# bamert/openGPC

Hardware: AMD Instinct MI355X
Metric: Mpix/s hashed+matched (1024x436 pair) (higher is better)
Workload: dtype u8; 1 GPU; BASELINE configs[1] pairs (1024x436, defaultZeroForest.txt, sparsematch settings: thr 5, epipolar, sort-match) in batches of 256 pairs per GPU per step (configs[3] sharding: pair i -> GPU i mod N); width=1024, height=436, tests=30, forest_type=0, parallelism=pairs-dp1, streams_per_gpu=1

## Files before the change

opengpc_amd/csrc/gpc_hip.hip:

```cpp
#include "../../include/gpc_hip.h"

#include <hip/hip_runtime.h>

#if defined(__SSE2__)
#include <emmintrin.h>
#endif
#include <sched.h>

#include <algorithm>
#include <cctype>
#include <condition_variable>
#include <cstdio>
#include <cstdlib>
#include <cstring>
#include <ctime>
#include <deque>
#include <map>
#include <utility>
#include <mutex>
#include <string>
#include <thread>
#include <vector>

#include "gpc_device.h"
// ... 98 lines not shown
class ExpandPool {
 public:
  ~ExpandPool() { stop(); }
  void start(int nthreads, const cpu_set_t* bind, const std::vector<cpu_set_t>* groups = nullptr) {
    if ((int)threads_.size() == nthreads) return;
    stop();
    quit_ = false;
    have_bind_ = bind != nullptr;
    if (bind) bind_ = *bind;
    groups_.clear();
    if (bind && groups) groups_ = *groups;
    cpus_.assign((size_t)nthreads, -1);
    for (int i = 0; i < nthreads; ++i)
      threads_.emplace_back([this, i] {
        if (!groups_.empty()) (void)sched_setaffinity(0, sizeof(cpu_set_t), &groups_[(size_t)i % groups_.size()]);
        else if (have_bind_) (void)sched_setaffinity(0, sizeof bind_, &bind_);
        run(i);
      });
  }
  void stop() {
    {
      std::lock_guard<std::mutex> g(m_);
      quit_ = true;
    }
    cv_.notify_all();
    for (auto& t : threads_) t.join();
    threads_.clear();
  }
  void push(const ExpandJob& j) {
    {
      std::lock_guard<std::mutex> g(m_);
      q_.push_back(j);
      ++pending_[j.slot & 7];
    }
    cv_.notify_one();
  }
  void wait_slot(int slot) {
    std::unique_lock<std::mutex> g(m_);
    done_.wait(g, [&] { return pending_[slot & 7] == 0; });
  }
  void wait_all() {
    for (int s = 0; s < 8; ++s) wait_slot(s);
  }
  int size() const { return (int)threads_.size(); }
  int worker_cpus(int* out, int cap) {
    std::lock_guard<std::mutex> g(m_);
    int n = 0;
    for (size_t i = 0; i < cpus_.size() && n < cap; ++i) out[n++] = cpus_[i];
    return (int)cpus_.size();
  }

 private:
  void run(int index);
  std::vector<std::thread> threads_;
  std::vector<int> cpus_;
  std::deque<ExpandJob> q_;
  std::mutex m_;
  std::condition_variable cv_, done_;
  int pending_[8] = {0, 0, 0, 0, 0, 0, 0, 0};
  bool quit_ = false;
  bool have_bind_ = false;
  cpu_set_t bind_;
  std::vector<cpu_set_t> groups_;
};

}

struct gpc_hip_ctx {
  int device = 0;
  hipStream_t own_stream = nullptr;
  hipStream_t stream = nullptr;
  hipStream_t s_in = nullptr, s_out = nullptr, s_cnt = nullptr;
  hipStream_t s_aux = nullptr;
  hipEvent_t e_fork = nullptr, e_join = nullptr;
  hipEvent_t e_flag = nullptr;
  hipEvent_t e_in[4] = {}, e_comp[4] = {}, e_cnt[4] = {}, e_out[4] = {};
  DevBuf packed;
  void* h_stage = nullptr;
  size_t h_stage_cap = 0;
  void* h_in = nullptr;
  size_t h_in_cap = 0;
  int32_t* h_cnt = nullptr;
  size_t h_cnt_cap = 0;
  ExpandPool pool;
  float stage_ms[4] = {0.f, 0.f, 0.f, 0.f};
  bool grad_is_bits = false;
  bool no_grad_bits = false;
  int upload_mode = 1;
  int direct_max = 2;
  bool have_node_cpus = false;
  cpu_set_t node_cpus;
  std::vector<cpu_set_t> node_l3;
  int numa_node = -1;
  struct Lane {
    hipStream_t s = nullptr;
    hipEvent_t e_in = nullptr, e_hash = nullptr, e_join = nullptr;
    DevBuf smooth, grad, codes, stats, jstate, staged, rowcnt;
    size_t jstate_granules = 0;
    uint32_t join_epoch = 0;
    bool grad_is_bits = false, used = false;
  };
  Lane lanes[2];
  int pipeline = 1, next_lane = 0;
  hipEvent_t dbg_wait_pre = nullptr, dbg_wait_hash = nullptr, dbg_rec_hash = nullptr, dbg_rec_join = nullptr;
  bool no_pair_packed = false;
  bool no_feeder = false;
  int fed_calls = 0;
  int chunk_pairs = 0;
  int expand_threads = 0;
  char err[256] = {0};

  bool naive = false;
  bool have_forest = false;
  GpcForestDev forest;
  GpcForestDev forest_naive;
  int forest_w = 0, forest_h = 0;
  gpc_filter_mask forest_src;
  int ngroups = 0;
  int gmax_tests = 0;
  bool gtau = false;
  DevBuf gforest_dev;
  DevBuf vstats, vcand, vout, vcnt, vncand, uplane, ublk, gdense;
  DevBuf all_rec, all_cnt;
  DevBuf stage;
  hipEvent_t e_stage[2] = {};
  DevBuf tr_plane, tr_pred, tr_blk;
  DevBuf cs_key, cs_idx, cs_cur, cs_start, cs_blk, cs_keep;
  DevBuf py_img, py_rec, py_cnt, py_plane, py_flags, py_blk;
  DevBuf sstats;

  DevBuf raw, smooth, grad, candmap, codes, staged, rowcnt, stats, out, counts, ncand, mask;
  DevBuf gkv;
  DevBuf gkeys[2], gvals[2], ghist, gmisc, hkeys[2], hvals[2], hrec;
  DevBuf gpart;
  int32_t* h_flag = nullptr;
  int no_partition = 0;
  int rows_per_chunk = 16;
  int gp_log2bins = 0;
  int ht_hint_w = 0, ht_hint_h = 0, ht_hint_lbits = 0;
  bool ht_no_half = false;
  int ht_mid = 0;
  int ht_lbits = 0;
  int gp_target = 2000;
  int flat_chunks = 0;
  DevBuf forest_dev;
  int hash_tall = -1;

  DevBuf jstate;
  size_t jstate_granules = 0;
  uint32_t join_epoch = 0;
  int32_t* h_err = nullptr;
  int32_t* d_err = nullptr;
  int no_fuse = 0;
  int fuse_always = 0;
  int fuse_wgs = 0;
  int fuse_min_pairs = 1;
  int pre_rows = 0;
  int fuse_shards = 0;
  int num_cus = 0;
  std::map<std::pair<const void*, size_t>, int> wgs_per_cu;
  std::map<const void*, int> dyn_lds;

  int hash_tpw = 0;
  int join_nt = 0;

  char launch_name[KID_COUNT][96] = {{0}};

  bool timing = false;
  unsigned timing_mask = 0xFFFFFFFFu;
  std::vector<TimedSpan> spans;
  std::vector<TimedSpan> free_spans;

  std::vector<gpc_hip_train_set*> train_sets;
  std::vector<gpc_hip_track_stream*> track_streams;
  uint64_t code_gen = 1;
  DevBuf ext_raw, ext_smooth, ext_grad, ext_groups;
  int extract_frames = 0;
  int seq_frames = 0;

  struct Resident {
    bool valid = false;
    const uint8_t *smooth = nullptr, *grad = nullptr;
    const int32_t* mask = nullptr;
    int n_mask = 0, W = 0, H = 0;
    bool naive = false;
    uint64_t fp = 0;
  };
  Resident res[2];
  int res_next = 0;
  DevBuf res_smooth, res_grad;
  size_t res_n = 0;
  int resident_mode = 1;
  int resident_hits = 0;
  uint8_t* h_xfer = nullptr;
  size_t h_xfer_cap = 0;
  uint8_t* h_pre = nullptr;
  size_t h_pre_cap = 0;
  int pre_slot = -1, pre_W = 0, pre_H = 0;
  bool pre_have_mask = false;
  hipEvent_t e_pre = nullptr;
  struct PendingMatch {
    bool active = false, direct = false, have_ncand = false;
    void* dev_out = nullptr;
    bool packed = false;
    size_t esz = 0;
    int cap_dev = 0, H = 0;
  } pend;
  bool debug = false;
  bool debug_plan = false;
};

struct gpc_hip_train_set {
  gpc_hip_ctx* owner = nullptr;
  int n = 0;
  long np = 0;
  uint8_t* planes = nullptr;
  uint8_t* flags = nullptr;
  int32_t* counts = nullptr;
  gpc::GpcSplit* d_cand = nullptr;
  size_t counts_cap = 0, cand_cap = 0;
  std::vector<int32_t> h_counts;
};

namespace {

std::mutex g_res_mu;
std::vector<gpc_hip_ctx*> g_ctxs;

#define HIPCHK(ctx, call)                                                              \
  do {                                                                                 \
    hipError_t e_ = (call);                                                            \
    if (e_ != hipSuccess) {                                                            \
      snprintf((ctx)->err, sizeof((ctx)->err), "%s failed: %s (%s:%d)", #call,        \
               hipGetErrorString(e_), __FILE__, __LINE__);                             \
      return GPC_E_HIP;                                                                \
    }                                                                                  \
  } while (0)

#define CHK(expr)                  \
  do {                             \
    int s_ = (expr);               \
    if (s_ != GPC_OK) return s_;   \
  } while (0)

double host_ms() {
  timespec ts;
  clock_gettime(CLOCK_MONOTONIC, &ts);
  return ts.tv_sec * 1e3 + ts.tv_nsec * 1e-6;
}

int ensure(gpc_hip_ctx* c, DevBuf& b, size_t bytes) {
  if (bytes <= b.cap) return GPC_OK;
  if (b.p) {
    HIPCHK(c, hipStreamSynchronize(c->stream));
    HIPCHK(c, hipFree(b.p));
    b.p = nullptr;
    b.cap = 0;
  }
  size_t want = bytes + bytes / 8 + 65536;
  HIPCHK(c, hipMalloc(&b.p, want));
  b.cap = want;
  return GPC_OK;
}

void release(DevBuf& b) {
  if (b.p) (void)hipFree(b.p);
  b.p = nullptr;
  b.cap = 0;
}

struct Timed {
  gpc_hip_ctx* c;
  TimedSpan s;
  bool on;
  Timed(gpc_hip_ctx* ctx, int kid) : c(ctx), on(ctx->timing && (kid >= 32 || ((ctx->timing_mask >> kid) & 1u))) {
    if (!on) return;
    if (!c->free_spans.empty()) {
      s = c->free_spans.back();
      c->free_spans.pop_back();
    } else {
      if (hipEventCreate(&s.a) != hipSuccess || hipEventCreate(&s.b) != hipSuccess) {
        on = false;
        return;
      }
    }
    s.kid = kid;
    (void)hipEventRecord(s.a, c->stream);
  }
  ~Timed() {
    if (!on) return;
    (void)hipEventRecord(s.b, c->stream);
    c->spans.push_back(s);
  }
};

int allow_dyn_lds(gpc_hip_ctx* c, const void* fn, size_t bytes) {
  int& have = c->dyn_lds[fn];
  if ((int)bytes <= have) return GPC_OK;
  HIPCHK(c, hipFuncSetAttribute(fn, hipFuncAttributeMaxDynamicSharedMemorySize, (int)bytes));
  have = (int)bytes;
  return GPC_OK;
}

int check_dims(int W, int H) {
  if (W <= 0 || H <= 0 || (W % 16) != 0) return GPC_E_INVALID;
  if (W < 2 * GPC_R + 16 || H < 2 * GPC_R + 4) return GPC_E_INVALID;
// ... 118 lines not shown
  const __m128i m16 = _mm_set1_epi32(0xFFFF);
#endif
  for (int y = y0; y < y1 && pos < limit; ++y) {
    const long cnt = rows[y];
    long n = cnt;
    if (pos + n > limit) n = limit - pos;
    long i = 0;
    auto one = [&](uint32_t v) {
      const int xl = (int)(v & 0xFFFFu), xr = (int)(v >> 16);
      out[pos].x = xl;
      out[pos].y = y;
      out[pos].d = (float)(xl - xr);
      ++pos;
    };
#if defined(__SSE2__)
    if (aligned) {
      for (; i < n && (pos & 3); ++i) one(src[i]);
      const __m128 Y = _mm_castsi128_ps(_mm_set1_epi32(y));
      for (; i + 4 <= n; i += 4, pos += 4) {
        const __m128i v = _mm_loadu_si128(reinterpret_cast<const __m128i*>(src + i));
        const __m128i xl = _mm_and_si128(v, m16);
        const __m128 X = _mm_castsi128_ps(xl);
        const __m128 D = _mm_cvtepi32_ps(_mm_sub_epi32(xl, _mm_srli_epi32(v, 16)));
        const __m128 t0 = _mm_castsi128_ps(_mm_unpacklo_epi32(xl, _mm_castps_si128(Y)));
        const __m128 t1 = _mm_castsi128_ps(_mm_unpackhi_epi32(xl, _mm_castps_si128(Y)));
        const __m128 a = _mm_shuffle_ps(t0, _mm_shuffle_ps(D, X, _MM_SHUFFLE(1, 1, 0, 0)), _MM_SHUFFLE(2, 0, 1, 0));
        const __m128 b = _mm_shuffle_ps(_mm_shuffle_ps(Y, D, _MM_SHUFFLE(1, 1, 0, 0)), t1, _MM_SHUFFLE(1, 0, 2, 0));
        const __m128 c = _mm_shuffle_ps(_mm_shuffle_ps(D, X, _MM_SHUFFLE(3, 3, 2, 2)),
                                        _mm_shuffle_ps(Y, D, _MM_SHUFFLE(3, 3, 0, 0)), _MM_SHUFFLE(2, 0, 2, 0));
        __m128i* o = reinterpret_cast<__m128i*>(out + pos);
        _mm_stream_si128(o, _mm_castps_si128(a));
        _mm_stream_si128(o + 1, _mm_castps_si128(b));
        _mm_stream_si128(o + 2, _mm_castps_si128(c));
      }
    }
#endif
    for (; i < n; ++i) one(src[i]);
    src += cnt;
  }
#if defined(__SSE2__)
  _mm_sfence();
#endif
}

void ExpandPool::run(int index) {
  for (;;) {
    ExpandJob j;
    {
      std::unique_lock<std::mutex> g(m_);
      cv_.wait(g, [&] { return quit_ || !q_.empty(); });
      if (q_.empty()) return;
      j = q_.front();
      q_.pop_front();
      cpus_[(size_t)index] = sched_getcpu();
    }
    if (j.copy_bytes) memcpy(j.copy_dst, j.copy_src, j.copy_bytes);
    else expand_rows(j.packed, j.rows, j.y0, j.y1, j.first, j.limit, j.out);
    {
      std::lock_guard<std::mutex> g(m_);
      if (--pending_[j.slot & 7] == 0) done_.notify_all();
    }
  }
}

int pow2_at_least(int v) {
  int p = 2;
  while (p < v) p <<= 1;
  return p;
}


bool next_tok(const char*& p, std::string& tok) {
  while (*p && isspace((unsigned char)*p)) ++p;
  if (!*p) return false;
  const char* s = p;
  while (*p && !isspace((unsigned char)*p)) ++p;
  tok.assign(s, p - s);
  return true;
}

bool next_int(const char*& p, int& v) {
  std::string tok;
  if (!next_tok(p, tok)) return false;
  char* end = nullptr;
  long l = strtol(tok.c_str(), &end, 10);
  if (end == tok.c_str()) return false;
  v = (int)l;
  return true;
}


int run_global_match(gpc_hip_ctx* c, int W, int H, int npairs, const gpc_settings* s, int mode, const uint8_t* d_cand,
                     void* d_out, int cap, int32_t* d_counts, int32_t* d_ncand, bool seq = false);
int run_hashtable_match(gpc_hip_ctx* c, int W, int H, int npairs, const gpc_settings* s, int mode, const uint8_t* d_cand,
                        void* d_out, int cap, int32_t* d_counts, int32_t* d_ncand, bool seq = false);

int run_preprocess(gpc_hip_ctx* c, const uint8_t* d_raw0, const uint8_t* d_raw1, int W, int H,
                   int npairs, int sides, int thr, bool gradbits = false, uint8_t* d_smooth_out = nullptr,
                   uint8_t* d_grad_out = nullptr, int32_t* d_stats = nullptr) {
  const int nimg = npairs * sides;
  const size_t n = (size_t)W * H;
  if (!d_smooth_out) {
    CHK(ensure(c, c->smooth, n * nimg));
    CHK(ensure(c, c->grad, n * nimg));
    d_smooth_out = (uint8_t*)c->smooth.p;
    d_grad_out = (uint8_t*)c->grad.p;
  } else {
    gradbits = false;
  }
  if (!d_stats) {
    CHK(ensure(c, c->stats, sizeof(int32_t) * GPC_STAT_STRIDE * nimg));
    d_stats = (int32_t*)c->stats.p;
  }
  const int thr_sq = c->naive ? (thr & 0xFF) * (thr & 0xFF) : (int)(int16_t)(uint16_t)((thr & 0xFF) * (thr & 0xFF));
  const int gx = (W / PP_PX + PP_TX - 1) / PP_TX;
  auto blocks_with = [&](int r) { return (long)gx * ((H + PP_TY * r - 1) / (PP_TY * r)) * nimg; };
  int rows = c->pre_rows;
  if (!rows) {
    static const int heights[] = {PP_ROWS, 10, 7, PP_ROWS_MID, 4, PP_ROWS_SMALL};
    const long places = 8l * (c->num_cus > 0 ? c->num_cus : 256);
    long best = -1;
    for (int r : heights) {
      const long cost = (blocks_with(r) + places - 1) / places * (r + 4);
      if (best < 0 || cost < best) { best = cost; rows = r; }
    }
  }
  dim3 grid(gx, (H + PP_TY * rows - 1) / (PP_TY * rows), nimg);
  Timed t(c, KID_PREPROCESS);
  c->grad_is_bits = gradbits && !c->naive && !c->no_grad_bits;
  snprintf(c->launch_name[KID_PREPROCESS], sizeof c->launch_name[0], "gpc::k_preprocess<%s, %d%s>", c->naive ? "true" : "false", rows,
           c->grad_is_bits ? ", true" : "");
#define LAUNCH_PRE(NAIVE, ROWS, BITS)                                                                        \
  hipLaunchKernelGGL((gpc::k_preprocess<NAIVE, ROWS, BITS>), grid, dim3(PP_TX * PP_TY), 0, c->stream, d_raw0, d_raw1, \
                     d_smooth_out, d_grad_out, W, H, sides, thr_sq, d_stats)
#define LAUNCH_PRE_ROWS(NAIVE, BITS)                                  \
  do {                                                                \
    if (rows == PP_ROWS) LAUNCH_PRE(NAIVE, PP_ROWS, BITS);            \
    else if (rows == 10) LAUNCH_PRE(NAIVE, 10, BITS);                 \
    else if (rows == 7) LAUNCH_PRE(NAIVE, 7, BITS);                   \
    else if (rows == PP_ROWS_MID) LAUNCH_PRE(NAIVE, PP_ROWS_MID, BITS); \
    else if (rows == 4) LAUNCH_PRE(NAIVE, 4, BITS);                   \
    else LAUNCH_PRE(NAIVE, PP_ROWS_SMALL, BITS);                      \
  } while (0)
  if (c->naive) LAUNCH_PRE_ROWS(true, false);
  else if (c->grad_is_bits) LAUNCH_PRE_ROWS(false, true);
  else LAUNCH_PRE_ROWS(false, false);
#undef LAUNCH_PRE_ROWS
#undef LAUNCH_PRE
  HIPCHK(c, hipGetLastError());
  return GPC_OK;
}

int run_hash(gpc_hip_ctx* c, const uint8_t* d_smooth, const uint8_t* d_grad, const uint8_t* d_cand,
             int W, int H, int nimg, bool dense, uint32_t* d_codes, int groups = 0, int gstep = 2, int32_t* d_stats = nullptr) {
  if (!c->have_forest) return GPC_E_NO_FOREST;
  const bool gbits = c->grad_is_bits && d_grad == (const uint8_t*)c->grad.p && !dense && !c->naive && d_cand == nullptr;
  const int slots = 2 * (c->num_cus > 0 ? c->num_cus : 256);
  const int gx = (W + HT_X - 1) / HT_X;
  int ty = HT_Y;
  {
    const long n32 = (long)gx * ((H - 2 * GPC_R + HT_Y - 1) / HT_Y) * nimg, n40 = (long)gx * ((H - 2 * GPC_R + HT_Y_TALL - 1) / HT_Y_TALL) * nimg;
    const long c32 = (n32 + slots - 1) / slots * (HT_Y + 2 * GPC_R), c40 = (n40 + slots - 1) / slots * (HT_Y_TALL + 2 * GPC_R);
    if (gbits && n32 < 2l * slots && c40 < c32) ty = HT_Y_TALL;
    if (gbits && c->hash_tall == 1) ty = HT_Y_TALL;
    if (c->hash_tall == 0) ty = HT_Y;
  }
  const int tiles_y = (H - 2 * GPC_R + ty - 1) / ty;
  int tpw = 1;
  if ((long)gx * tiles_y * nimg >= 2l * slots) {
    double best = 1e30;
    for (int t = 2; t <= 16 && t <= tiles_y; ++t) {
      const long per_col = (tiles_y + t - 1) / t, ncol = (long)gx * nimg;
      const long nwg = per_col * ncol;
      if (nwg * 8 < (long)slots * 7) break;
      const int rem = tiles_y - (int)(per_col - 1) * t;
      const long n_full = (per_col - 1) * ncol, n_rem = ncol;
      const long full_rounds = n_full / slots, full_left = n_full % slots;
      double chain = (double)full_rounds * (t + 0.4);
      long short_left = n_rem;
      if (full_left) {
        const long free_places = slots - full_left;
        const long fit = free_places * (long)((t + 0.4) / (rem + 0.4));
        short_left = n_rem > fit ? n_rem - fit : 0;
        chain += t + 0.4;
      }
      chain += (double)((short_left + slots - 1) / slots) * (rem + 0.4);
      if (chain < best - 1e-9) { best = chain; tpw = t; }
    }
  }
  if (c->hash_tpw > 0) tpw = c->hash_tpw < tiles_y ? c->hash_tpw : tiles_y;
  dim3 grid(gx, (tiles_y + tpw - 1) / tpw, nimg);
  const long nwg_all = (long)grid.x * grid.y * grid.z;
  const int last_from = nwg_all > slots ? (int)(nwg_all - slots) : 0;
  Timed t(c, KID_HASH);
  const bool tau = groups > 0 ? c->gtau : c->forest.type != 0;
  int32_t* st = d_stats ? d_stats : (int32_t*)c->stats.p;
  if (groups > 0) {
    const GpcForestDev* gf = (const GpcForestDev*)c->gforest_dev.p;
    snprintf(c->launch_name[KID_HASH], sizeof c->launch_name[0], "gpc::k_hash_groups<%s, %s, %s, %s, %d>", tau ? "true" : "false",
             dense ? "true" : "false", c->naive ? "true" : "false", gbits ? "true" : "false", ty);
#define LAUNCH_HASH_G(TAU, DENSE, NAIVE, GB, TY, FD)                                                                       \
  hipLaunchKernelGGL((gpc::k_hash_groups<TAU, DENSE, NAIVE, GB, TY>), grid, dim3(HT_THREADS), 0, c->stream, d_smooth, d_grad, \
                     d_cand, d_codes, W, H, gf + (FD) * GPC_MAX_GROUPS, st, tpw, last_from, groups, gstep)
    if (gbits) {
      if (ty == HT_Y_TALL) {
        if (tau) LAUNCH_HASH_G(true, false, false, true, HT_Y_TALL, 2); else LAUNCH_HASH_G(false, false, false, true, HT_Y_TALL, 2);
      } else {
        if (tau) LAUNCH_HASH_G(true, false, false, true, HT_Y, 0); else LAUNCH_HASH_G(false, false, false, true, HT_Y, 0);
      }
    } else if (c->naive) {
      if (tau && dense) LAUNCH_HASH_G(true, true, true, false, HT_Y, 1);
      else if (tau) LAUNCH_HASH_G(true, false, true, false, HT_Y, 1);
      else if (dense) LAUNCH_HASH_G(false, true, true, false, HT_Y, 1);
      else LAUNCH_HASH_G(false, false, true, false, HT_Y, 1);
    } else {
      if (tau && dense) LAUNCH_HASH_G(true, true, false, false, HT_Y, 0);
      else if (tau) LAUNCH_HASH_G(true, false, false, false, HT_Y, 0);
      else if (dense) LAUNCH_HASH_G(false, true, false, false, HT_Y, 0);
      else LAUNCH_HASH_G(false, false, false, false, HT_Y, 0);
    }
#undef LAUNCH_HASH_G
    HIPCHK(c, hipGetLastError());
    return GPC_OK;
  }
  snprintf(c->launch_name[KID_HASH], sizeof c->launch_name[0], "gpc::k_hash<%s, %s, %s, %s, %d>", tau ? "true" : "false",
           dense ? "true" : "false", c->naive ? "true" : "false", gbits ? "true" : "false", ty);
#define LAUNCH_HASH(TAU, DENSE, NAIVE)                                                                    \
  hipLaunchKernelGGL((gpc::k_hash<TAU, DENSE, NAIVE>), grid, dim3(HT_THREADS), 0, c->stream, d_smooth, d_grad, \
                     d_cand, d_codes, W, H, (const GpcForestDev*)c->forest_dev.p + (NAIVE ? 1 : 0), st, tpw, last_from)
  if (gbits) {
#define LAUNCH_HASH_BITS(TAU, TY, FD)                                                                                      \
  hipLaunchKernelGGL((gpc::k_hash<TAU, false, false, true, TY>), grid, dim3(HT_THREADS), 0, c->stream, d_smooth, d_grad, \
                     d_cand, d_codes, W, H, (const GpcForestDev*)c->forest_dev.p + FD, st, tpw, last_from)
    if (ty == HT_Y_TALL) {
      if (tau) LAUNCH_HASH_BITS(true, HT_Y_TALL, 2); else LAUNCH_HASH_BITS(false, HT_Y_TALL, 2);
    } else {
      if (tau) LAUNCH_HASH_BITS(true, HT_Y, 0); else LAUNCH_HASH_BITS(false, HT_Y, 0);
    }
#undef LAUNCH_HASH_BITS
  } else if (c->naive) {
    if (tau && dense) LAUNCH_HASH(true, true, true);
    else if (tau) LAUNCH_HASH(true, false, true);
    else if (dense) LAUNCH_HASH(false, true, true);
    else LAUNCH_HASH(false, false, true);
  } else {
    if (tau && dense) LAUNCH_HASH(true, true, false);
    else if (tau) LAUNCH_HASH(true, false, false);
    else if (dense) LAUNCH_HASH(false, true, false);
    else LAUNCH_HASH(false, false, false);
  }
#undef LAUNCH_HASH
  HIPCHK(c, hipGetLastError());
  return GPC_OK;
}

int code_bits(const gpc_hip_ctx* c) {
  const int T = c->ngroups > 1 ? c->gmax_tests : c->forest.num_tests;
  if (c->naive) return T;
  return T <= 8 ? T : T - 1;
}

bool wide_codes(const gpc_hip_ctx* c) { return c->naive && (c->ngroups > 1 ? c->gmax_tests : c->forest.num_tests) == 32; }

struct JoinPlan {
  int nt, spt, log2s;
  size_t lds;
};

JoinPlan plan_join(const gpc_hip_ctx* c, int W) {
  JoinPlan p;
  p.spt = 1;
  p.nt = 256;
  while (p.spt * p.nt < W && p.spt < 4) p.spt <<= 1;
  while (p.spt * p.nt < W && p.nt < 1024) p.nt <<= 1;
  if (c->join_nt && 4 * c->join_nt >= W) {
    p.nt = c->join_nt;
    p.spt = 1;
    while (p.spt * p.nt < W) p.spt <<= 1;
  }
  while (p.spt * p.nt < W && p.spt < 16) p.spt <<= 1;
  p.log2s = 1;
  while ((1 << p.log2s) < p.nt * p.spt || ((1 << p.log2s) < 2 * (W - 2 * GPC_R) && p.log2s < 14)) ++p.log2s;
  p.lds = ((size_t)8 * ((1u << p.log2s) + 1) + 15) / 16 * 16;
  return p;
}

int check_join_err(gpc_hip_ctx* c) {
#ifdef RJ_DBG_COUNT
  if (c->h_err && c->h_err[1]) {
    fprintf(stderr, "[RJ_DBG_COUNT] look-backs %d, windows with a row that had not published %d, displaced keys that met their copy %d\n", c->h_err[1], c->h_err[2], c->h_err[3]);
    c->h_err[1] = c->h_err[2] = c->h_err[3] = 0;
  }
#endif
  if (c->h_err) {
    const int32_t ep = __atomic_exchange_n(c->h_err, 0, __ATOMIC_ACQ_REL);
    if (ep) {
      snprintf(c->err, sizeof(c->err), "k_row_join_fused: a row waited too long for the rows before it in fused launch %d of this "
               "context (%u launched so far): THAT launch's supports are not to be used; a call that reports this at its start "
               "has queued nothing itself", ep, c->join_epoch);
      return GPC_E_HIP;
    }
  }
  return GPC_OK;
}

int join_shards(const gpc_hip_ctx* c, int npairs) {
  if (c->fuse_shards > 0) return npairs < c->fuse_shards ? npairs : c->fuse_shards;
  return join_shards_auto(npairs);
}

int ensure_join_state(gpc_hip_ctx* c, size_t granules) {
  const size_t tk_bytes = sizeof(uint32_t) * RJ_SHARDS * RJ_TICKET_STRIDE;
  if (!c->h_err) {
    HIPCHK(c, hipHostMalloc((void**)&c->h_err, 64, hipHostMallocMapped));
    memset(c->h_err, 0, 64);
    HIPCHK(c, hipHostGetDevicePointer((void**)&c->d_err, c->h_err, 0));
  }
  if (granules > c->jstate_granules || c->join_epoch >= (1u << 30) - 2u) {
    CHK(ensure(c, c->jstate, tk_bytes + sizeof(unsigned long long) * granules));
    HIPCHK(c, hipMemsetAsync(c->jstate.p, 0, c->jstate.cap, c->stream));
    c->jstate_granules = (c->jstate.cap - tk_bytes) / sizeof(unsigned long long);
    c->join_epoch = 0;
  }
  return GPC_OK;
}

int ensure_flag_event(gpc_hip_ctx* c) {
  if (!c->e_flag) HIPCHK(c, hipEventCreateWithFlags(&c->e_flag, hipEventDisableTiming));
  return GPC_OK;
}

int ensure_aux_stream(gpc_hip_ctx* c) {
  if (c->s_aux) return GPC_OK;
  HIPCHK(c, hipStreamCreateWithFlags(&c->s_aux, hipStreamNonBlocking));
  HIPCHK(c, hipEventCreateWithFlags(&c->e_fork, hipEventDisableTiming));
  HIPCHK(c, hipEventCreateWithFlags(&c->e_join, hipEventDisableTiming));
  return GPC_OK;
}

int run_match(gpc_hip_ctx* c, int W, int H, int npairs, const gpc_settings* s, int mode, const uint8_t* d_cand,
              void* d_out, int cap, int32_t* d_counts, int32_t* d_ncand, const PackedOut* po = nullptr, bool seq = false) {
  const int apply_filter = (mode != 1);
  if (mode == 2 && (s->use_hashtable || !s->epipolar_mode || !po)) return GPC_E_UNSUPPORTED;
  if (seq && (mode == 2 || po)) return GPC_E_UNSUPPORTED;
  if (s->use_hashtable) return run_hashtable_match(c, W, H, npairs, s, mode, d_cand, d_out, cap, d_counts, d_ncand, seq);
  if (s->epipolar_mode) {
    CHK(ensure(c, c->staged, sizeof(uint32_t) * (size_t)W * H * npairs));
    CHK(ensure(c, c->rowcnt, sizeof(int32_t) * (size_t)H * npairs * 2));
    int disp_high = s->disp_high;
    if (apply_filter && s->vertical_tolerance < 0) disp_high = -1;
    const JoinPlan jp = plan_join(c, W);
    if (jp.nt * jp.spt < W) return GPC_E_UNSUPPORTED;
    const size_t flds = RJF_LDS_BYTES(jp.nt * jp.spt);
    bool fuse = !seq && !c->no_fuse && npairs >= c->fuse_min_pairs && jp.spt <= 4 && jp.nt * jp.spt <= 4096 &&
                !(po && po->totals) && (long)npairs * (H - 2 * GPC_R) < (1l << 31) - 65536;
    if (fuse && !c->fuse_always) {
      const long lds_wgs = (long)(160 * 1024 / (flds + 64)), wave_wgs = 32 / (jp.nt / 64);
      const long resident = (long)c->num_cus * (lds_wgs < wave_wgs ? lds_wgs : wave_wgs);
      const long rows_total = (long)npairs * (H - 2 * GPC_R);
      fuse = rows_total >= 4 * resident || (W >= 2048 && rows_total >= 3 * resident);
    }
    if (fuse) {
      const int nrows = H - 2 * GPC_R;
      CHK(check_join_err(c));
      CHK(ensure_join_state(c, (size_t)npairs * nrows));
      const size_t lds = flds;
      gpc::RjfArgs a;
      memset(&a, 0, sizeof a);
      a.codes = (const uint32_t*)c->codes.p;
      a.cand = d_cand;
      a.img_stats = (const int32_t*)c->stats.p;
      a.tickets = (uint32_t*)c->jstate.p;
      a.status = (unsigned long long*)((uint32_t*)c->jstate.p + RJ_SHARDS * RJ_TICKET_STRIDE);
      a.err = c->d_err;
      a.out = d_out;
      a.counts = d_counts;
      a.ncand = d_ncand;
      a.rows_out = po ? po->rows : nullptr;
      a.packed_stride = po ? po->packed_stride : 0l;
      a.rows_stride = po ? po->rows_stride : 0l;
      a.W = W;
      a.H = H;
      a.disp_high = disp_high;
      a.apply_filter = apply_filter;
      a.epoch = ++c->join_epoch;
      a.npairs = npairs;
      a.mode = mode;
      a.cap = cap;
      Timed t(c, KID_ROW_JOIN);
      const bool wide = wide_codes(c);
      snprintf(c->launch_name[KID_ROW_JOIN], sizeof c->launch_name[0], "gpc::k_row_join_fused<%d, %d, %s>", jp.spt, jp.nt,
               wide ? "true" : "false");
      c->launch_name[KID_GATHER_ROWS][0] = 0;
#define LAUNCH_RJF(SPT, NT, WIDE)                                                                               \
  do {                                                                                                          \
    const void* fn_ = reinterpret_cast<const void*>(gpc::k_row_join_fused<SPT, NT, WIDE>);                      \
    int& per_cu = c->wgs_per_cu[std::make_pair(fn_, lds)];                                                      \
    if (per_cu == 0) {                                                                                          \
      if (lds > 48 * 1024) CHK(allow_dyn_lds(c, fn_, lds));                                                     \
      HIPCHK(c, hipOccupancyMaxActiveBlocksPerMultiprocessor(&per_cu, fn_, NT, lds));                           \
      if (per_cu < 1) per_cu = 1;                                                                               \
    }                                                                                                           \
     \
    long nwg = c->fuse_wgs > 0 ? c->fuse_wgs : (long)((c->pipeline > 1 && per_cu > 1) ? per_cu - 1 : per_cu) * c->num_cus; \
    if (nwg > (long)npairs * nrows) nwg = (long)npairs * nrows;                                                 \
               \
    int nsh = join_shards(c, npairs);                                                                           \
    if (nsh > nwg) nsh = (int)nwg;                                                                              \
    a.nshards = nsh;                                                                                            \
    if (c->debug) fprintf(stderr, "[gpc_hip] k_row_join_fused<%d, %d>: %d workgroups per CU by the occupancy API, %ld workgroups, %d shards, %zu B of LDS\n", SPT, NT, per_cu, nwg, nsh, lds); \
    const GpcJoinSplit sp_ = make_join_split(npairs, nsh);                                                      \
    a.n_hi = sp_.n_hi;                                                                                          \
    for (int k_ = 0; k_ < 2; ++k_) {                                                                            \
      a.ps[k_] = sp_.ps[k_];                                                                                    \
      a.ps_magic[k_] = sp_.ps_magic[k_];                                                                        \
      a.ps_sh[k_] = sp_.ps_sh[k_];                                                                              \
    }                                                                                                           \
    hipLaunchKernelGGL((gpc::k_row_join_fused<SPT, NT, WIDE>), dim3((unsigned)nwg), dim3(NT), lds, c->stream, a); \
  } while (0)
#define LAUNCH_RJF_W(SPT, NT) do { if (wide) LAUNCH_RJF(SPT, NT, true); else LAUNCH_RJF(SPT, NT, false); } while (0)
#define LAUNCH_RJF_S(NT)                      \
  switch (jp.spt) {                           \
    case 1: LAUNCH_RJF_W(1, NT); break;       \
    case 2: LAUNCH_RJF_W(2, NT); break;       \
    default: LAUNCH_RJF_W(4, NT); break;      \
  }
      if (jp.nt == 1024) { LAUNCH_RJF_S(1024) }
      else if (jp.nt == 512) { LAUNCH_RJF_S(512) }
      else { LAUNCH_RJF_S(256) }
#undef LAUNCH_RJF_S
#undef LAUNCH_RJF_W
#undef LAUNCH_RJF
      HIPCHK(c, hipGetLastError());
      return GPC_OK;
    }
    {
      Timed t(c, KID_ROW_JOIN);
      const int rpw = 1;
      const dim3 jgrid((H - 2 * GPC_R + rpw - 1) / rpw, npairs);
      const bool wide = wide_codes(c);
      snprintf(c->launch_name[KID_ROW_JOIN], sizeof c->launch_name[0], "gpc::k_row_join%s<%d, %d, %s>", seq ? "_seq" : "",
               jp.spt, jp.nt, wide ? "true" : "false");
#define LAUNCH_JOIN_K(K, SPT, NT, WIDE)                                                                       \
  do {                                                                                                        \
    const void* fn_ = reinterpret_cast<const void*>(gpc::K<SPT, NT, WIDE>);                                   \
    if (jp.lds > 48 * 1024) CHK(allow_dyn_lds(c, fn_, jp.lds));                                               \
    hipLaunchKernelGGL((gpc::K<SPT, NT, WIDE>), jgrid, dim3(NT), jp.lds, c->stream,                           \
                       (const uint32_t*)c->codes.p, d_cand, W, H, disp_high, apply_filter,                    \
                       (const int32_t*)c->stats.p, (uint32_t*)c->staged.p, (int32_t*)c->rowcnt.p, jp.log2s,   \
                       rpw, gpc::RjVirt());                                                    \
  } while (0)
#define LAUNCH_JOIN(SPT, NT, WIDE) \
  do { if (seq) LAUNCH_JOIN_K(k_row_join_seq, SPT, NT, WIDE); else LAUNCH_JOIN_K(k_row_join, SPT, NT, WIDE); } while (0)
#define LAUNCH_JOIN_W(SPT, NT) do { if (wide) LAUNCH_JOIN(SPT, NT, true); else LAUNCH_JOIN(SPT, NT, false); } while (0)
#define LAUNCH_JOIN_S(NT)                      \
  switch (jp.spt) {                            \
    case 1: LAUNCH_JOIN_W(1, NT); break;       \
    case 2: LAUNCH_JOIN_W(2, NT); break;       \
    default: LAUNCH_JOIN_W(4, NT); break;      \
  }
      if (jp.nt == 1024) {
        if (jp.spt == 16) LAUNCH_JOIN_W(16, 1024);
        else if (jp.spt == 8) LAUNCH_JOIN_W(8, 1024);
        else LAUNCH_JOIN_S(1024)
      } else if (jp.nt == 512) { LAUNCH_JOIN_S(512) }
      else { LAUNCH_JOIN_S(256) }
#undef LAUNCH_JOIN_S
#undef LAUNCH_JOIN_W
#undef LAUNCH_JOIN
#undef LAUNCH_JOIN_K
      HIPCHK(c, hipGetLastError());
    }
    {
      Timed t(c, KID_GATHER_ROWS);
      snprintf(c->launch_name[KID_GATHER_ROWS], sizeof c->launch_name[0], "gpc::k_gather_rows");
      if (po && po->totals)
        hipLaunchKernelGGL(gpc::k_pair_totals, dim3(npairs), dim3(RM_THREADS), 0, c->stream, (const int32_t*)c->rowcnt.p, H,
                           po->totals);
      const int gr = ((long)((H - 2 * GPC_R + GR_ROWS - 1) / GR_ROWS) * npairs >= 2048) ? GR_ROWS : 1;
      hipLaunchKernelGGL(gpc::k_gather_rows, dim3((H - 2 * GPC_R + gr - 1) / gr, npairs), dim3(RM_THREADS), 0, c->stream,
                         (const uint32_t*)c->staged.p, (const int32_t*)c->rowcnt.p, W, H, mode, d_out,
                         cap, d_counts, (const int32_t*)c->stats.p, d_ncand, gr, po ? po->rows : nullptr,
                         po ? po->packed_stride : 0l, po ? po->rows_stride : 0l,
                         po ? (const int32_t*)po->totals : (const int32_t*)nullptr);
      HIPCHK(c, hipGetLastError());
    }
    return GPC_OK;
  }
  return run_global_match(c, W, H, npairs, s, mode, d_cand, d_out, cap, d_counts, d_ncand, seq);
}

struct GlobalPlan {
  int nmax, nblk, nmblk;
  gpc::GpcBatchStrides bs;
  int32_t *hist, *blkcnt, *gmisc, *rowcnt;
  size_t esz;
};

int plan_global(gpc_hip_ctx* c, int W, int H, int npairs, int mode, int cap, bool hashtable, GlobalPlan& g, bool seq) {
  const size_t n = (size_t)W * H;
  g.nmax = 2 * (W - 2 * GPC_R) * (H - 2 * GPC_R);
  g.nblk = (g.nmax + GS_TILE - 1) / GS_TILE;
  g.nmblk = (g.nmax + RM_THREADS - 1) / RM_THREADS;
  g.esz = mode == 0 ? sizeof(gpc_support) : sizeof(gpc_correspondence);
  const size_t recs = (size_t)g.nmax * npairs;
  for (int i = 0; i < 2; ++i) {
    CHK(ensure(c, c->gkeys[i], sizeof(uint32_t) * recs));
    CHK(ensure(c, c->gvals[i], sizeof(uint32_t) * recs));
    if (hashtable) {
      CHK(ensure(c, c->hkeys[i], sizeof(uint32_t) * recs));
      CHK(ensure(c, c->hvals[i], sizeof(uint32_t) * recs));
    }
  }
  if (hashtable) CHK(ensure(c, c->hrec, 2 * sizeof(uint32_t) * recs));
  CHK(ensure(c, c->ghist, sizeof(int32_t) * ((size_t)256 * g.nblk + g.nmblk) * npairs));
  CHK(ensure(c, c->gmisc, sizeof(int32_t) * GM_STRIDE * npairs));
  CHK(ensure(c, c->rowcnt, sizeof(int32_t) * (size_t)H * 2 * npairs));
  g.hist = (int32_t*)c->ghist.p;
  g.blkcnt = g.hist + (size_t)256 * g.nblk * npairs;
  g.gmisc = (int32_t*)c->gmisc.p;
  g.rowcnt = (int32_t*)c->rowcnt.p;
  g.bs.codes = (long)((seq ? 1 : 2) * n);
  g.bs.recs = g.nmax;
  g.bs.hist = (long)256 * g.nblk;
  g.bs.blk = g.nmblk;
  g.bs.out = (long)cap * (long)g.esz;
  g.bs.rows = 2 * H;
  return GPC_OK;
}

int radix_passes(gpc_hip_ctx* c, const GlobalPlan& g, int npairs, uint32_t* keys[2], uint32_t* vals[2], int passes) {
  for (int pass = 0; pass < passes; ++pass) {
    const int src = pass & 1, dst = src ^ 1;
    hipLaunchKernelGGL(gpc::k_g_hist, dim3(g.nblk, npairs), dim3(GS_THREADS), 0, c->stream,
                       (const uint32_t*)keys[src], (const int32_t*)g.gmisc, 8 * pass, g.hist, g.nblk, g.bs);
    hipLaunchKernelGGL(gpc::k_g_scan, dim3(1, npairs), dim3(1024), 0, c->stream, g.hist, 256 * g.nblk, g.bs.hist);
    hipLaunchKernelGGL(gpc::k_g_scatter, dim3(g.nblk, npairs), dim3(GS_THREADS), 0, c->stream,
                       (const uint32_t*)keys[src], (const uint32_t*)vals[src], keys[dst], vals[dst],
                       (const int32_t*)g.gmisc, 8 * pass, (const int32_t*)g.hist, g.nblk, g.bs);
  }
  HIPCHK(c, hipGetLastError());
  return GPC_OK;
}

void launch_radix_records(gpc_hip_ctx* c, const GlobalPlan& g, int W, int H, int npairs, const uint8_t* d_cand, uint32_t* keys,
                          uint32_t* vals) {
  const uint32_t* codes = (const uint32_t*)c->codes.p;
  const uint8_t* wcand = wide_codes(c) ? d_cand : nullptr;
  const int32_t* stats = (const int32_t*)c->stats.p;
  const dim3 rgrid(H - 2 * GPC_R, 2, npairs);
  hipLaunchKernelGGL(gpc::k_g_rowcount, rgrid, dim3(RM_THREADS), 0, c->stream, codes, wcand, W, H, g.rowcnt, stats, g.gmisc, g.bs);
  hipLaunchKernelGGL(gpc::k_g_build, rgrid, dim3(RM_THREADS), 0, c->stream, codes, wcand, W, H, (const int32_t*)g.rowcnt, stats,
                     keys, vals, g.gmisc, g.bs);
}

void name_join_launch(gpc_hip_ctx* c, const char* kernel, bool list) {
  char* n = c->launch_name[KID_GLOBAL_MATCH];
  const size_t at = strlen(n);
  snprintf(n + at, sizeof c->launch_name[0] - at, "%s%s%s", at ? " + " : "", kernel, list ? "[list]" : "");
}

struct CodeRangePlan {
  int32_t overflow;
  int32_t max_parts;
  int32_t max_bin_side;
  int32_t max_list;
};
struct BucketCheck {
  int32_t overflow;
  int32_t max_bin;
  int32_t max_pair;
  int32_t max_list;
};
template <class Words>
Words plan_words(const gpc_hip_ctx* c) {
  static_assert(sizeof(Words) == 4 * sizeof(int32_t), "a planner leaves four words");
  Words w;
  memcpy(&w, c->h_flag, sizeof w);
  return w;
}

struct PartIo {
  const uint32_t* codes;
  const uint8_t* wcand;
// ... 640 lines not shown
}

namespace {

int run_group_match(gpc_hip_ctx* c, const uint8_t* d_sm, const uint8_t* d_gr, const uint8_t* d_cand_hash, int W, int H,
                    int npairs, const gpc_settings* s, int mode, const uint8_t* d_cand, void* d_out, long cap,
                    int32_t* d_counts, int32_t* d_ncand) {
  if (s->use_hashtable) return GPC_E_UNSUPPORTED;
  const int G = c->ngroups;
  const size_t n = (size_t)W * H;
  const int npv = npairs * G;
  const size_t esz = mode == 0 ? sizeof(gpc_support) : sizeof(gpc_correspondence);
  const long vcap = (long)(W - 2 * GPC_R) * (H - 2 * GPC_R) + 1;
  CHK(ensure(c, c->codes, sizeof(uint32_t) * n * 2 * npv));
  CHK(ensure(c, c->vstats, sizeof(int32_t) * GPC_STAT_STRIDE * 2 * npv));
  CHK(ensure(c, c->vout, esz * (size_t)vcap * npv));
  CHK(ensure(c, c->vcnt, sizeof(int32_t) * npv));
  CHK(ensure(c, c->vncand, sizeof(int32_t) * 2 * npv));
  hipLaunchKernelGGL(gpc::k_stats_init, dim3((2 * npv + 63) / 64), dim3(64), 0, c->stream, (int32_t*)c->vstats.p, 2 * npv);
  std::swap(c->stats, c->vstats);
  int st = run_hash(c, d_sm, d_gr, d_cand_hash, W, H, 2 * npairs, false, (uint32_t*)c->codes.p, G, 2);
  const uint8_t* vc = d_cand;
  if (st == GPC_OK && wide_codes(c) && d_cand) {
    st = ensure(c, c->vcand, 2 * n * npv);
    for (int p = 0; p < npairs && st == GPC_OK; ++p)
      for (int g = 0; g < G && st == GPC_OK; ++g)
        if (hipMemcpyAsync((uint8_t*)c->vcand.p + (size_t)(p * G + g) * 2 * n, d_cand + (size_t)p * 2 * n, 2 * n,
                           hipMemcpyDeviceToDevice, c->stream) != hipSuccess)
          st = GPC_E_HIP;
    vc = (const uint8_t*)c->vcand.p;
  }
  if (st == GPC_OK)
    st = run_match(c, W, H, npv, s, mode, vc, c->vout.p, (int)vcap, (int32_t*)c->vcnt.p, (int32_t*)c->vncand.p);
  std::swap(c->stats, c->vstats);
  CHK(st);
  const int nchunk = (int)((vcap + UN_CHUNK - 1) / UN_CHUNK);
  CHK(ensure(c, c->uplane, sizeof(uint32_t) * n * npv));
  CHK(ensure(c, c->ublk, sizeof(int32_t) * (size_t)nchunk * npv));
  Timed t(c, KID_GROUP_UNION);
  snprintf(c->launch_name[KID_GROUP_UNION], sizeof c->launch_name[0], "gpc::k_group_union<%s>", mode == 0 ? "false" : "true");
  HIPCHK(c, hipMemsetAsync(c->uplane.p, 0xFF, sizeof(uint32_t) * n * npv, c->stream));
  const dim3 sgrid(nchunk < 512 ? nchunk : 512, npv), cgrid(nchunk, npv);
#define UNION_LAUNCH(CORR)                                                                                                  \
  do {                                                                                                                     \
    typedef gpc::UnRec<CORR> R_;                                                                                           \
    const R_* vo_ = (const R_*)c->vout.p;                                                                                  \
    hipLaunchKernelGGL((gpc::k_group_union_scatter<CORR>), sgrid, dim3(UN_THREADS), 0, c->stream, vo_,                     \
                       (const int32_t*)c->vcnt.p, vcap, W, H, (uint32_t*)c->uplane.p, G);                                  \
    hipLaunchKernelGGL((gpc::k_group_union_count<CORR>), cgrid, dim3(UN_THREADS), 0, c->stream, vo_,                       \
                       (const int32_t*)c->vcnt.p, vcap, W, H, (const uint32_t*)c->uplane.p, G, (int32_t*)c->ublk.p, nchunk); \
    hipLaunchKernelGGL(gpc::k_group_union_scan, dim3(npairs), dim3(1024), 0, c->stream, (int32_t*)c->ublk.p, nchunk, G,    \
                       d_counts, d_ncand, (const int32_t*)c->vstats.p);                                                    \
    hipLaunchKernelGGL((gpc::k_group_union<CORR>), cgrid, dim3(UN_THREADS), 0, c->stream, vo_, (const int32_t*)c->vcnt.p,  \
                       vcap, W, H, (const uint32_t*)c->uplane.p, G, (const int32_t*)c->ublk.p, nchunk, (R_*)d_out, cap);   \
  } while (0)
  if (mode == 0) UNION_LAUNCH(false);
  else UNION_LAUNCH(true);
#undef UNION_LAUNCH
  HIPCHK(c, hipGetLastError());
  return GPC_OK;
}

}


extern "C" {

int gpc_hip_abi_version(void) { return GPC_HIP_ABI_VERSION; }

const char* gpc_hip_status_string(int status) {
  switch (status) {
    case GPC_OK: return "ok";
    case GPC_E_INVALID: return "invalid argument";
    case GPC_E_NO_DEVICE: return "no usable HIP device (gfx950 required)";
    case GPC_E_HIP: return "HIP runtime error";
    case GPC_E_CAPACITY: return "output capacity too small";
    case GPC_E_NO_FOREST: return "no forest set";
    case GPC_E_FOREST_RANGE: return "forest test offset outside the 27x27 patch";
    case GPC_E_IO: return "forest file could not be read";
    case GPC_E_UNSUPPORTED: return "unsupported setting on the HIP path";
    default: return "unknown status";
  }
}

int gpc_hip_device_count(int* count) {
  if (!count) return GPC_E_INVALID;
  int n = 0;
  if (hipGetDeviceCount(&n) != hipSuccess) {
    *count = 0;
    return GPC_E_NO_DEVICE;
  }
  *count = n;
  return GPC_OK;
}

int gpc_hip_create(int device, gpc_hip_ctx** out) {
  if (!out) return GPC_E_INVALID;
  *out = nullptr;
  int n = 0;
  if (hipGetDeviceCount(&n) != hipSuccess || n <= 0 || device < 0 || device >= n) return GPC_E_NO_DEVICE;
  if (hipSetDevice(device) != hipSuccess) return GPC_E_NO_DEVICE;
  hipDeviceProp_t prop;
  if (hipGetDeviceProperties(&prop, device) != hipSuccess) return GPC_E_NO_DEVICE;
  if (strncmp(prop.gcnArchName, "gfx950", 6) != 0) return GPC_E_NO_DEVICE;
  gpc_hip_ctx* c = new gpc_hip_ctx();
  c->device = device;
  if (hipStreamCreateWithFlags(&c->own_stream, hipStreamNonBlocking) != hipSuccess) {
    delete c;
    return GPC_E_NO_DEVICE;
  }
  c->stream = c->own_stream;
  const char* ht = getenv("GPC_HIP_HASH_TPW");
  if (ht && atoi(ht) > 0 && atoi(ht) <= 64) c->hash_tpw = atoi(ht);
  c->no_partition = getenv("GPC_HIP_NO_PARTITION") != nullptr;
  c->flat_chunks = getenv("GPC_HIP_FLAT_CHUNKS") != nullptr;
  if (const char* e = getenv("GPC_HIP_GP_TARGET")) {
    const int v = atoi(e);
    if (v >= 256 && v <= 3500) c->gp_target = v;
  }
  if (const char* e = getenv("GPC_HIP_GP_LOG2BINS")) {
    const int v = atoi(e);
    if (v >= 8 && v <= 11) c->gp_log2bins = v;
  }
  c->ht_no_half = getenv("GPC_HIP_HT_NO_HALF") != nullptr;
  if (const char* e = getenv("GPC_HIP_HT_MID")) {
    const int v = atoi(e);
    if (v >= HM_CAP && v <= 64) c->ht_mid = v;
  }
  if (const char* e = getenv("GPC_HIP_HT_LBITS")) {
    const int v = atoi(e);
    if (v >= 7 && v <= 10) c->ht_lbits = v;
  }
  if (const char* e = getenv("GPC_HIP_ROWS_PER_CHUNK")) {
    const int v = atoi(e);
    if (v >= 1 && v <= 64) c->rows_per_chunk = v;
  }
  if (const char* e = getenv("GPC_HIP_DIRECT_MAX")) {
    const int v = atoi(e);
    if (v >= 0 && v <= 4096) c->direct_max = v;
  }
  const char* ck = getenv("GPC_HIP_CHUNK");
  if (ck && atoi(ck) > 0 && atoi(ck) <= 1024) c->chunk_pairs = atoi(ck);
  if (const char* e = getenv("GPC_HIP_SEQ_FRAMES")) {
    const int v = atoi(e);
    if (v >= 2 && v <= 1024) c->seq_frames = v;
  }
  const char* et = getenv("GPC_HIP_EXPAND_THREADS");
  if (et && atoi(et) > 0 && atoi(et) <= 64) c->expand_threads = atoi(et);
  if (const char* e = getenv("GPC_HIP_UPLOAD")) c->upload_mode = atoi(e);
  c->no_grad_bits = getenv("GPC_HIP_NO_GRAD_BITS") != nullptr;
  c->no_feeder = getenv("GPC_HIP_NO_FEEDER") != nullptr;
  c->no_pair_packed = getenv("GPC_HIP_NO_PAIR_PACKED") != nullptr;
  c->no_fuse = getenv("GPC_HIP_NO_FUSE") != nullptr;
  if (const char* e = getenv("GPC_HIP_HASH_TALL")) c->hash_tall = atoi(e) ? 1 : 0;
  if (const char* e = getenv("GPC_HIP_PRE_ROWS")) {
    const int v = atoi(e);
    if (v == PP_ROWS || v == 10 || v == 7 || v == PP_ROWS_MID || v == 4 || v == PP_ROWS_SMALL) c->pre_rows = v;
  }
  c->fuse_always = getenv("GPC_HIP_FUSE_ALWAYS") != nullptr;
  if (const char* e = getenv("GPC_HIP_FUSE_WGS")) {
    const int v = atoi(e);
    if (v >= 1 && v <= 65536) c->fuse_wgs = v;
  }
  if (const char* e = getenv("GPC_HIP_FUSE_SHARDS")) {
    const int v = atoi(e);
    if (v >= 1 && v <= RJ_SHARDS) c->fuse_shards = v;
  }
  if (const char* e = getenv("GPC_HIP_FUSE_MIN_PAIRS")) {
    const int v = atoi(e);
    if (v >= 1) c->fuse_min_pairs = v;
  }
  if (const char* e = getenv("GPC_HIP_RESIDENT")) {
    const int v = atoi(e);
    if (v >= 0 && v <= 2) c->resident_mode = v;
  }
  if (const char* e = getenv("GPC_HIP_EXTRACT_FRAMES")) {
    const int v = atoi(e);
    if (v >= 1) c->extract_frames = v;
  }
  c->debug = getenv("GPC_HIP_DEBUG") != nullptr;
  c->debug_plan = getenv("GPC_HIP_DEBUG_PLAN") != nullptr;
  c->num_cus = prop.multiProcessorCount;
  find_gpu_node_cpus(c);
  const char* jn = getenv("GPC_HIP_JOIN_NT");
  if (jn && (atoi(jn) == 256 || atoi(jn) == 512 || atoi(jn) == 1024)) c->join_nt = atoi(jn);
  {
    std::lock_guard<std::mutex> g(g_res_mu);
    g_ctxs.push_back(c);
  }
  *out = c;
  return GPC_OK;
}

int gpc_hip_destroy(gpc_hip_ctx* c) {
  if (!c) return GPC_E_INVALID;
  {
    std::lock_guard<std::mutex> g(g_res_mu);
    for (size_t k = 0; k < g_ctxs.size(); ++k)
      if (g_ctxs[k] == c) { g_ctxs.erase(g_ctxs.begin() + k); break; }
  }
  (void)hipSetDevice(c->device);
  (void)drain_lanes(c);
  (void)hipStreamSynchronize(c->stream);
  const int pending_err = check_join_err(c);
  if (pending_err != GPC_OK) fprintf(stderr, "gpc_hip_destroy: %s\n", c->err);
  DevBuf* bufs[] = {&c->raw, &c->smooth, &c->grad, &c->candmap, &c->codes, &c->staged, &c->rowcnt,
                    &c->stats, &c->out, &c->counts, &c->ncand, &c->mask, &c->gkeys[0], &c->gkeys[1],
                    &c->gvals[0], &c->gvals[1], &c->ghist, &c->gmisc, &c->hkeys[0], &c->hkeys[1],
                    &c->hvals[0], &c->hvals[1], &c->hrec, &c->forest_dev, &c->packed, &c->gpart, &c->jstate, &c->gkv,
                    &c->res_smooth, &c->res_grad, &c->ext_raw, &c->ext_smooth, &c->ext_grad, &c->ext_groups,
                    &c->sstats, &c->all_rec, &c->all_cnt, &c->stage, &c->tr_plane, &c->tr_pred, &c->tr_blk,
                    &c->cs_key, &c->cs_idx, &c->cs_cur, &c->cs_start, &c->cs_blk, &c->cs_keep,
                    &c->py_img, &c->py_rec, &c->py_cnt, &c->py_plane, &c->py_flags, &c->py_blk};
  while (!c->train_sets.empty()) (void)gpc_hip_train_set_destroy(c, c->train_sets.back());
  while (!c->track_streams.empty()) (void)gpc_hip_track_stream_destroy(c, c->track_streams.back());
  for (DevBuf* b : bufs) release(*b);
  for (auto& s : c->spans) { (void)hipEventDestroy(s.a); (void)hipEventDestroy(s.b); }
  for (auto& s : c->free_spans) { (void)hipEventDestroy(s.a); (void)hipEventDestroy(s.b); }
  if (c->s_in) {
    (void)hipStreamDestroy(c->s_in);
    (void)hipStreamDestroy(c->s_out);
    (void)hipStreamDestroy(c->s_cnt);
    for (int i = 0; i < 4; ++i) {
      (void)hipEventDestroy(c->e_in[i]);
      (void)hipEventDestroy(c->e_comp[i]);
      (void)hipEventDestroy(c->e_cnt[i]);
      (void)hipEventDestroy(c->e_out[i]);
    }
  }
  if (c->e_flag) (void)hipEventDestroy(c->e_flag);
  if (c->e_pre) (void)hipEventDestroy(c->e_pre);
  for (hipEvent_t e : c->e_stage)
    if (e) (void)hipEventDestroy(e);
  for (auto& l : c->lanes) {
    if (l.s) {
      (void)hipStreamSynchronize(l.s);
      (void)hipStreamDestroy(l.s);
      (void)hipEventDestroy(l.e_in);
      (void)hipEventDestroy(l.e_hash);
      (void)hipEventDestroy(l.e_join);
    }
    DevBuf* lb[] = {&l.smooth, &l.grad, &l.codes, &l.stats, &l.jstate, &l.staged, &l.rowcnt};
    for (DevBuf* b : lb) release(*b);
  }
  if (c->s_aux) {
    (void)hipStreamDestroy(c->s_aux);
    (void)hipEventDestroy(c->e_fork);
    (void)hipEventDestroy(c->e_join);
  }
  c->pool.stop();
  if (c->h_stage) (void)hipHostFree(c->h_stage);
  if (c->h_in) (void)hipHostFree(c->h_in);
  if (c->h_cnt) (void)hipHostFree(c->h_cnt);
  if (c->h_pre) (void)hipHostFree(c->h_pre);
  if (c->h_xfer) (void)hipHostFree(c->h_xfer);
  if (c->h_flag) (void)hipHostFree(c->h_flag);
  if (c->h_err) (void)hipHostFree(c->h_err);
  if (c->own_stream) (void)hipStreamDestroy(c->own_stream);
  delete c;
  return pending_err;
}

const char* gpc_hip_last_error(const gpc_hip_ctx* c) { return c ? c->err : "null context"; }

int gpc_hip_set_stream(gpc_hip_ctx* c, void* hip_stream) {
  if (!c) return GPC_E_INVALID;
  c->stream = hip_stream ? (hipStream_t)hip_stream : c->own_stream;
  return GPC_OK;
}

int gpc_hip_synchronize(gpc_hip_ctx* c) {
  if (!c) return GPC_E_INVALID;
  CHK(drain_lanes(c));
  HIPCHK(c, hipStreamSynchronize(c->stream));
  return check_join_err(c);
}

int gpc_hip_reserve(gpc_hip_ctx* c, int W, int H, int max_pairs) {
  if (!c || max_pairs <= 0) return GPC_E_INVALID;
  CHK(check_dims(W, H));
  HIPCHK(c, hipSetDevice(c->device));
  const size_t n = (size_t)W * H;
  const int nimg = 2 * max_pairs;
  const int G = c->ngroups > 1 ? c->ngroups : 1;
  CHK(ensure(c, c->raw, n * nimg));
  CHK(ensure(c, c->smooth, n * nimg));
  CHK(ensure(c, c->grad, n * nimg));
  CHK(ensure(c, c->codes, sizeof(uint32_t) * n * nimg * G));
  if (G > 1) {
    CHK(ensure(c, c->vstats, sizeof(int32_t) * GPC_STAT_STRIDE * nimg * G));
    CHK(ensure(c, c->vcnt, sizeof(int32_t) * max_pairs * G));
    CHK(ensure(c, c->vncand, sizeof(int32_t) * nimg * G));
    CHK(ensure(c, c->uplane, sizeof(uint32_t) * n * max_pairs * G));
  }
  CHK(ensure(c, c->staged, sizeof(uint32_t) * n * max_pairs));
  CHK(ensure(c, c->rowcnt, sizeof(int32_t) * (size_t)H * nimg));
  CHK(ensure(c, c->stats, sizeof(int32_t) * GPC_STAT_STRIDE * nimg));
  CHK(ensure(c, c->counts, sizeof(int32_t) * nimg));
  CHK(ensure(c, c->ncand, sizeof(int32_t) * nimg));
  return GPC_OK;
}

int gpc_hip_set_arithmetic(gpc_hip_ctx* c, int mode) {
  if (!c || (mode != GPC_ARITH_SSE && mode != GPC_ARITH_NAIVE)) return GPC_E_INVALID;
  if (c->naive != (mode == GPC_ARITH_NAIVE)) ++c->code_gen;
  c->naive = (mode == GPC_ARITH_NAIVE);
// ... 526 lines not shown
    d_sm = (const uint8_t*)c->smooth.p;
    d_gr = (const uint8_t*)c->grad.p;
    d_cand = d_cm;
  }
  c->grad_is_bits = false;
  c->pend.dev_out = nullptr;
  if (groups) {
    const long cap_u = (long)c->ngroups * ((long)(W - 2 * GPC_R) * (H - 2 * GPC_R)) + 1;
    CHK(ensure(c, c->gdense, esz * (size_t)cap_u));
    CHK(run_group_match(c, d_sm, d_gr, resident ? nullptr : d_cand, W, H, 1, s, mode, d_cand, c->gdense.p, cap_u, d_cnt,
                        nullptr));
    cap_dev = (int)std::min(cap_u, (long)INT32_MAX);
    c->pend.dev_out = c->gdense.p;
  } else {
  hipLaunchKernelGGL(gpc::k_stats_init, dim3(1), dim3(64), 0, c->stream, (int32_t*)c->stats.p, 2);
  CHK(run_hash(c, d_sm, d_gr, resident ? nullptr : d_cand, W, H, 2, false, (uint32_t*)c->codes.p));
  if (packed) {
    const PackedOut po = {reinterpret_cast<int32_t*>(d_arena), (long)cap_dev, (long)H};
    CHK(run_match(c, W, H, 1, s, 2, d_cand, d_arena + rows_bytes, cap_dev, d_cnt, nullptr, &po));
  } else {
    CHK(run_match(c, W, H, 1, s, mode, d_cand, d_out, cap_dev, d_cnt, nullptr));
  }
  }
  c->pend.active = true;
  c->pend.direct = direct_out != nullptr;
  c->pend.have_ncand = false;
  c->pend.packed = packed;
  c->pend.esz = esz;
  c->pend.cap_dev = cap_dev;
  c->pend.H = H;
  return GPC_OK;
}

static int match_fetch(gpc_hip_ctx* c, void* out, int cap, int* n_out, int* ncl, int* ncr) {
  if (!c || !c->pend.active || !n_out || cap < 0 || (cap > 0 && !out)) return GPC_E_INVALID;
  HIPCHK(c, hipStreamSynchronize(c->stream));
  CHK(check_join_err(c));
  const int32_t cnt = c->h_cnt[0];
  *n_out = cnt;
  if (c->pend.have_ncand) {
    if (ncl) *ncl = c->h_cnt[1];
    if (ncr) *ncr = c->h_cnt[2];
  }
  int ncopy = cnt < cap ? cnt : cap;
  if (ncopy > c->pend.cap_dev) ncopy = c->pend.cap_dev;
  if (c->pend.dev_out && ncopy > 0) {
    const size_t bytes = c->pend.esz * (size_t)ncopy;
    uint8_t* d_arena = nullptr;
    CHK(xfer_reserve(c, bytes, &d_arena));
    HIPCHK(c, hipMemcpyAsync(c->h_xfer, c->pend.dev_out, bytes, hipMemcpyDeviceToHost, c->stream));
    HIPCHK(c, hipStreamSynchronize(c->stream));
    const bool par = bytes >= 256 * 1024;
    if (par) CHK(ensure_pool(c));
    host_copy(c, out, c->h_xfer, bytes, par);
    if (par) host_copy_wait(c);
  } else if (c->pend.packed && ncopy > 0) {
    const int H = c->pend.H;
    const int32_t* rows = reinterpret_cast<const int32_t*>(c->h_xfer);
    const uint32_t* words = reinterpret_cast<const uint32_t*>(c->h_xfer + pad16(sizeof(int32_t) * (size_t)H));
    const bool par = ncopy >= 32 * 1024;
    if (par) CHK(ensure_pool(c));
    const int parts = par ? (c->pool.size() > 1 ? c->pool.size() : 1) : 1;
    long first = 0;
    for (int q = 0; q < parts; ++q) {
      const int y0 = GPC_R + (int)((long)(H - 2 * GPC_R) * q / parts), y1 = GPC_R + (int)((long)(H - 2 * GPC_R) * (q + 1) / parts);
      if (first < ncopy && y1 > y0) {
        if (par) c->pool.push(ExpandJob{words, rows, H, y0, y1, (int)first, ncopy, static_cast<gpc_support*>(out), 6});
        else expand_rows(words, rows, y0, y1, first, ncopy, static_cast<gpc_support*>(out));
      }
      for (int y = y0; y < y1; ++y) first += rows[y];
    }
    if (par) host_copy_wait(c);
  } else if (!c->pend.direct && ncopy > 0) {
    const size_t bytes = c->pend.esz * (size_t)ncopy;
    const bool par = bytes >= 256 * 1024;
    if (par) CHK(ensure_pool(c));
    host_copy(c, out, c->h_xfer, bytes, par);
    if (par) host_copy_wait(c);
  }
  return (cnt > cap || cnt > c->pend.cap_dev) ? GPC_E_CAPACITY : GPC_OK;
}

static int match_preprocessed(gpc_hip_ctx* c, const uint8_t* smoothL, const uint8_t* gradL,
                              const int32_t* maskL, int nL, const uint8_t* smoothR, const uint8_t* gradR,
                              const int32_t* maskR, int nR, int W, int H, const gpc_settings* s, int mode,
                              void* out, int cap, int* n_out) {
  if (!n_out || cap < 0 || (cap > 0 && !out)) return GPC_E_INVALID;
  const size_t esz = mode == 0 ? sizeof(gpc_support) : sizeof(gpc_correspondence);
  void* dv = (c && cap > 0 && (uint64_t)cap * esz < (1ull << 32)) ? device_view_of_host(out) : nullptr;
  CHK(match_preprocessed_begin(c, smoothL, gradL, maskL, nL, smoothR, gradR, maskR, nR, W, H, s, mode, cap, dv));
  const int st = match_fetch(c, out, cap, n_out, nullptr, nullptr);
  c->pend.active = false;
  return st;
}

int gpc_hip_rectified_match(gpc_hip_ctx* c, const uint8_t* smoothL, const uint8_t* gradL,
                            const int32_t* maskL, int nL, const uint8_t* smoothR, const uint8_t* gradR,
                            const int32_t* maskR, int nR, int W, int H, const gpc_settings* s,
                            gpc_support* out, int cap, int* n_out) {
  return match_preprocessed(c, smoothL, gradL, maskL, nL, smoothR, gradR, maskR, nR, W, H, s, 0, out, cap, n_out);
}

int gpc_hip_stereo_match(gpc_hip_ctx* c, const uint8_t* smoothL, const uint8_t* gradL,
                         const int32_t* maskL, int nL, const uint8_t* smoothR, const uint8_t* gradR,
                         const int32_t* maskR, int nR, int W, int H, const gpc_settings* s,
                         gpc_correspondence* out, int cap, int* n_out) {
  return match_preprocessed(c, smoothL, gradL, maskL, nL, smoothR, gradR, maskR, nR, W, H, s, 1, out, cap, n_out);
}

int gpc_hip_rectified_match_begin(gpc_hip_ctx* c, const uint8_t* smoothL, const uint8_t* gradL, const int32_t* maskL, int nL,
                                  const uint8_t* smoothR, const uint8_t* gradR, const int32_t* maskR, int nR, int W, int H,
                                  const gpc_settings* s) {
  return match_preprocessed_begin(c, smoothL, gradL, maskL, nL, smoothR, gradR, maskR, nR, W, H, s, 0, (nL < nR ? nL : nR) + 1, nullptr);
}

int gpc_hip_stereo_match_begin(gpc_hip_ctx* c, const uint8_t* smoothL, const uint8_t* gradL, const int32_t* maskL, int nL,
                               const uint8_t* smoothR, const uint8_t* gradR, const int32_t* maskR, int nR, int W, int H,
                               const gpc_settings* s) {
  return match_preprocessed_begin(c, smoothL, gradL, maskL, nL, smoothR, gradR, maskR, nR, W, H, s, 1, (nL < nR ? nL : nR) + 1, nullptr);
}

int gpc_hip_match_fetch(gpc_hip_ctx* c, void* out, int cap, int* n_out, int* n_cand_l, int* n_cand_r) {
  return match_fetch(c, out, cap, n_out, n_cand_l, n_cand_r);
}


int gpc_hip_match_batch_device(gpc_hip_ctx* c, const uint8_t* d_rawL, const uint8_t* d_rawR, int W, int H,
                               int npairs, const gpc_settings* s, gpc_support* d_out, int cap_per_pair,
                               int32_t* d_counts, int32_t* d_ncand) {
  if (!c || !d_rawL || !d_rawR || !d_out || !d_counts || npairs <= 0 || cap_per_pair <= 0) return GPC_E_INVALID;
  CHK(check_settings(s));
  CHK(check_dims(W, H));
  CHK(forest_matches(c, W, H));
  HIPCHK(c, hipSetDevice(c->device));
  const size_t n = (size_t)W * H;
  if (c->ngroups > 1) {
    if (c->pipeline > 1 || s->use_hashtable) return GPC_E_UNSUPPORTED;
    CHK(run_preprocess(c, d_rawL, d_rawR, W, H, npairs, 2, s->gradient_threshold, true));
    return run_group_match(c, (const uint8_t*)c->smooth.p, (const uint8_t*)c->grad.p, nullptr, W, H, npairs, s, 0,
                           (const uint8_t*)c->grad.p, d_out, cap_per_pair, d_counts, d_ncand);
  }
  if (c->pipeline > 1 && s->epipolar_mode && !s->use_hashtable) {
    CHK(ensure_lanes(c));
    gpc_hip_ctx::Lane& lane = c->lanes[c->next_lane];
    gpc_hip_ctx::Lane& other = c->lanes[c->next_lane ^ 1];
    c->next_lane ^= 1;
    HIPCHK(c, hipEventRecord(lane.e_in, c->stream));
    HIPCHK(c, hipStreamWaitEvent(lane.s, lane.e_in, 0));
    if (other.used) HIPCHK(c, hipStreamWaitEvent(lane.s, other.e_hash, 0));
    LaneScope in(c, lane);
    lane.used = true;
    CHK(ensure(c, c->codes, sizeof(uint32_t) * n * 2 * npairs));
    CHK(run_preprocess(c, d_rawL, d_rawR, W, H, npairs, 2, s->gradient_threshold, true));
    CHK(run_hash(c, (const uint8_t*)c->smooth.p, (const uint8_t*)c->grad.p, nullptr, W, H, 2 * npairs, false, (uint32_t*)c->codes.p));
    HIPCHK(c, hipEventRecord(lane.e_hash, c->stream));
    CHK(run_match(c, W, H, npairs, s, 0, (const uint8_t*)c->grad.p, d_out, cap_per_pair, d_counts, d_ncand));
    HIPCHK(c, hipEventRecord(lane.e_join, c->stream));
    return GPC_OK;
  }
  if (c->pipeline > 1) CHK(drain_lanes(c));
  CHK(ensure(c, c->codes, sizeof(uint32_t) * n * 2 * npairs));
  if (c->dbg_wait_pre) HIPCHK(c, hipStreamWaitEvent(c->stream, c->dbg_wait_pre, 0));
  CHK(run_preprocess(c, d_rawL, d_rawR, W, H, npairs, 2, s->gradient_threshold, true));
  if (c->dbg_wait_hash) HIPCHK(c, hipStreamWaitEvent(c->stream, c->dbg_wait_hash, 0));
  CHK(run_hash(c, (const uint8_t*)c->smooth.p, (const uint8_t*)c->grad.p, nullptr, W, H, 2 * npairs, false,
               (uint32_t*)c->codes.p));
  if (c->dbg_rec_hash) HIPCHK(c, hipEventRecord(c->dbg_rec_hash, c->stream));
  CHK(run_match(c, W, H, npairs, s, 0, (const uint8_t*)c->grad.p, d_out, cap_per_pair, d_counts, d_ncand));
  if (c->dbg_rec_join) HIPCHK(c, hipEventRecord(c->dbg_rec_join, c->stream));
  return GPC_OK;
}

int gpc_hip_set_pipeline(gpc_hip_ctx* c, int lanes) {
  if (!c || (lanes != 1 && lanes != 2)) return GPC_E_INVALID;
  if (lanes == 2 && c->ngroups > 1) return GPC_E_UNSUPPORTED;
  HIPCHK(c, hipSetDevice(c->device));
  CHK(drain_lanes(c));
  HIPCHK(c, hipStreamSynchronize(c->stream));
  c->pipeline = lanes;
  return GPC_OK;
}

int gpc_hip_pipeline_join(gpc_hip_ctx* c) {
  if (!c) return GPC_E_INVALID;
  for (auto& l : c->lanes)
    if (l.s && l.used) HIPCHK(c, hipStreamWaitEvent(c->stream, l.e_join, 0));
  return GPC_OK;
}

int gpc_hip_debug_pipeline_events(gpc_hip_ctx* c, void* wait_before_preprocess, void* wait_before_hash, void* record_after_hash,
                                  void* record_after_join) {
  if (!c) return GPC_E_INVALID;
  c->dbg_wait_pre = (hipEvent_t)wait_before_preprocess;
  c->dbg_wait_hash = (hipEvent_t)wait_before_hash;
  c->dbg_rec_hash = (hipEvent_t)record_after_hash;
  c->dbg_rec_join = (hipEvent_t)record_after_join;
  return GPC_OK;
}

static int batch_streams(gpc_hip_ctx* c) {
  if (c->s_in) return GPC_OK;
  HIPCHK(c, hipStreamCreateWithFlags(&c->s_in, hipStreamNonBlocking));
  HIPCHK(c, hipStreamCreateWithFlags(&c->s_out, hipStreamNonBlocking));
  HIPCHK(c, hipStreamCreateWithFlags(&c->s_cnt, hipStreamNonBlocking));
  for (int i = 0; i < 4; ++i) {
    HIPCHK(c, hipEventCreateWithFlags(&c->e_in[i], hipEventDisableTiming));
    HIPCHK(c, hipEventCreateWithFlags(&c->e_comp[i], hipEventDisableTiming));
    HIPCHK(c, hipEventCreateWithFlags(&c->e_cnt[i], hipEventDisableTiming));
    HIPCHK(c, hipEventCreateWithFlags(&c->e_out[i], hipEventDisableTiming));
  }
  return GPC_OK;
}

static int match_batch_unpacked(gpc_hip_ctx* c, const uint8_t* rawL, const uint8_t* rawR, int W, int H, int npairs,
                                const gpc_settings* s, gpc_support* out, int cap, int32_t* counts, int32_t* ncand) {
  if (!c || !rawL || !rawR || !out || !counts || npairs <= 0 || cap <= 0) return GPC_E_INVALID;
  CHK(check_settings(s));
  CHK(check_dims(W, H));
  CHK(forest_matches(c, W, H));
  HIPCHK(c, hipSetDevice(c->device));
  const size_t n = (size_t)W * H;
  const int chunk = npairs >= 8 ? (npairs >= 32 ? 8 : npairs / 4) : npairs;
  const int nch = (npairs + chunk - 1) / chunk;
  CHK(ensure(c, c->raw, 2 * 2 * n * chunk));
  CHK(ensure(c, c->out, sizeof(gpc_support) * (size_t)cap * npairs));
  CHK(ensure(c, c->counts, sizeof(int32_t) * npairs));
  CHK(ensure(c, c->ncand, sizeof(int32_t) * 2 * npairs));
  CHK(batch_streams(c));
  CHK(pinned_counts(c, npairs));
  const bool bounce = !device_view_of_host(rawL) || !device_view_of_host(rawR);
  const bool land = !device_view_of_host(out);
  if (bounce || land) CHK(ensure_pool(c));
  if (bounce) {
    const size_t need = 2 * 2 * n * (size_t)chunk;
    if (need > c->h_in_cap) {
      HIPCHK(c, hipStreamSynchronize(c->s_in));
      if (c->h_in) HIPCHK(c, hipHostFree(c->h_in));
      c->h_in = nullptr;
      c->h_in_cap = 0;
      HIPCHK(c, hipHostMalloc(&c->h_in, need, hipHostMallocDefault));
      c->h_in_cap = need;
    }
  }
  const size_t slot_bytes = sizeof(gpc_support) * (size_t)cap * chunk;
  if (land && 2 * slot_bytes > c->h_stage_cap) {
    c->pool.wait_all();
    HIPCHK(c, hipStreamSynchronize(c->s_out));
    if (c->h_stage) HIPCHK(c, hipHostFree(c->h_stage));
    c->h_stage = nullptr;
    c->h_stage_cap = 0;
    HIPCHK(c, hipHostMalloc(&c->h_stage, 2 * slot_bytes, hipHostMallocDefault));
    c->h_stage_cap = 2 * slot_bytes;
  }
  int32_t* hc = c->h_cnt;
  int32_t* hn = c->h_cnt + npairs;
  int status = GPC_OK;
  auto collect = [&](int k) -> int {
    const int p0 = k * chunk, pc = (p0 + chunk <= npairs) ? chunk : npairs - p0;
    HIPCHK(c, hipEventSynchronize(c->e_cnt[k & 1]));
    memcpy(counts + p0, hc + p0, sizeof(int32_t) * pc);
    if (ncand) memcpy(ncand + 2 * p0, hn + 2 * p0, sizeof(int32_t) * 2 * pc);
    if (land) c->pool.wait_slot(k & 1);
    gpc_support* lslot = land ? reinterpret_cast<gpc_support*>((uint8_t*)c->h_stage + (size_t)(k & 1) * slot_bytes) : nullptr;
    for (int p = p0; p < p0 + pc; ++p) {
      const int ncopy = counts[p] < cap ? counts[p] : cap;
      if (counts[p] > cap) status = GPC_E_CAPACITY;
      if (ncopy > 0)
        HIPCHK(c, hipMemcpyAsync(land ? lslot + (size_t)(p - p0) * cap : out + (size_t)p * cap,
                                 (gpc_support*)c->out.p + (size_t)p * cap, sizeof(gpc_support) * (size_t)ncopy,
                                 hipMemcpyDeviceToHost, c->s_out));
    }
    if (land) HIPCHK(c, hipEventRecord(c->e_out[k & 1], c->s_out));
    return GPC_OK;
  };
  auto deliver = [&](int k) -> int {
    if (!land) return GPC_OK;
    const int p0 = k * chunk, pc = (p0 + chunk <= npairs) ? chunk : npairs - p0;
    HIPCHK(c, hipEventSynchronize(c->e_out[k & 1]));
    const gpc_support* lslot = reinterpret_cast<const gpc_support*>((uint8_t*)c->h_stage + (size_t)(k & 1) * slot_bytes);
    for (int p = p0; p < p0 + pc; ++p) {
      const int ncopy = counts[p] < cap ? counts[p] : cap;
      const size_t bytes = sizeof(gpc_support) * (size_t)ncopy, step = 256 * 1024;
      for (size_t at = 0; at < bytes; at += step) {
        ExpandJob j = {};
        j.slot = k & 1;
        j.copy_src = reinterpret_cast<const uint8_t*>(lslot + (size_t)(p - p0) * cap) + at;
        j.copy_dst = reinterpret_cast<uint8_t*>(out + (size_t)p * cap) + at;
        j.copy_bytes = at + step <= bytes ? step : bytes - at;
        c->pool.push(j);
      }
    }
    return GPC_OK;
  };
  for (int k = 0; k < nch; ++k) {
    const int slot = k & 1, p0 = k * chunk, pc = (p0 + chunk <= npairs) ? chunk : npairs - p0;
    uint8_t* d_l = (uint8_t*)c->raw.p + (size_t)slot * 2 * n * chunk;
    uint8_t* d_r = d_l + n * chunk;
    if (k >= 2) HIPCHK(c, hipStreamWaitEvent(c->s_in, c->e_comp[slot], 0));
    const uint8_t *srcL = rawL + (size_t)p0 * n, *srcR = rawR + (size_t)p0 * n;
    if (bounce) {
      uint8_t* bl = (uint8_t*)c->h_in + (size_t)slot * 2 * n * chunk;
      uint8_t* br = bl + n * chunk;
      if (k >= 2) HIPCHK(c, hipEventSynchronize(c->e_in[slot]));
      const size_t bytes = n * pc, step = 256 * 1024;
      for (int side = 0; side < 2; ++side)
        for (size_t at = 0; at < bytes; at += step) {
          ExpandJob j = {};
          j.slot = 7;
          j.copy_src = (side ? srcR : srcL) + at;
          j.copy_dst = (side ? br : bl) + at;
          j.copy_bytes = at + step <= bytes ? step : bytes - at;
          c->pool.push(j);
        }
      c->pool.wait_slot(7);
      srcL = bl;
      srcR = br;
    }
    HIPCHK(c, hipMemcpyAsync(d_l, srcL, n * pc, hipMemcpyHostToDevice, c->s_in));
    HIPCHK(c, hipMemcpyAsync(d_r, srcR, n * pc, hipMemcpyHostToDevice, c->s_in));
    HIPCHK(c, hipEventRecord(c->e_in[slot], c->s_in));
    HIPCHK(c, hipStreamWaitEvent(c->stream, c->e_in[slot], 0));
// ... 1363 lines not shown
extern "C++" {
template <bool CORR>
static int pyr_match(gpc_hip_ctx* c, const uint8_t* d_a, const uint8_t* d_b, int W, int H, int npairs, int levels,
                     const gpc_settings* s, void* d_out, int cap, int32_t* d_counts, int32_t* d_level_counts, int32_t* d_ncand) {
  int32_t ws[GPC_MAX_PYRAMID_LEVELS], hs[GPC_MAX_PYRAMID_LEVELS];
  CHK(pyr_usable(c, s, W, H, levels, ws, hs));
  if (npairs > 65535) return GPC_E_UNSUPPORTED;
  if (levels > 1) {
    CHK(gpc::pyr_down_check(d_a, d_out, W, H, CORR ? npairs + 1 : npairs));
    if (!CORR) CHK(gpc::pyr_down_check(d_b, d_out, W, H, npairs));
  }
  HIPCHK(c, hipSetDevice(c->device));
  if (c->pipeline > 1) CHK(drain_lanes(c));
  StrictScope strict(c);
  const int nimg = CORR ? npairs + 1 : npairs;
  const size_t ncs = CORR ? (size_t)nimg : 2 * (size_t)npairs;
  auto match = [&](int l, const uint8_t* a, const uint8_t* b, void* rec, int rcap, int32_t* cnt) -> int {
    const gpc_settings sl = gpc::pyr_level_settings(*s, l);
    int32_t* nc = d_ncand ? d_ncand + (size_t)l * ncs : nullptr;
    LevelScope level(c, ws[l], hs[l]);
    if (CORR) return gpc_hip_match_sequence_device(c, a, ws[l], hs[l], nimg, &sl, (gpc_correspondence*)rec, rcap, cnt, nc);
    return gpc_hip_match_batch_device(c, a, b, ws[l], hs[l], npairs, &sl, (gpc_support*)rec, rcap, cnt, nc);
  };
  if (levels == 1) {
    CHK(match(0, d_a, d_b, d_out, cap, d_counts));
    HIPCHK(c, hipMemcpyAsync(d_level_counts, d_counts, sizeof(int32_t) * (size_t)npairs, hipMemcpyDeviceToDevice, c->stream));
    return GPC_OK;
  }
  const size_t esz = sizeof(gpc::PyRec<CORR>);
  size_t img_at[GPC_MAX_PYRAMID_LEVELS] = {0}, rec_at[GPC_MAX_PYRAMID_LEVELS] = {0}, img_bytes = 0, rec_bytes = 0;
  int32_t caps[GPC_MAX_PYRAMID_LEVELS];
  for (int l = 0; l < levels; ++l) {
    caps[l] = (int32_t)gpc::pyr_level_cap(ws[l], hs[l]);
    rec_at[l] = rec_bytes;
    rec_bytes += pad16(esz * (size_t)caps[l] * npairs);
    if (!l) continue;
    img_at[l] = img_bytes;
    img_bytes += pad16((size_t)ws[l] * hs[l] * nimg) * (CORR ? 1 : 2);
  }
  CHK(ensure(c, c->py_img, img_bytes));
  CHK(ensure(c, c->py_rec, rec_bytes));
  CHK(ensure(c, c->py_cnt, sizeof(int32_t) * (size_t)levels * npairs));
  const void* d_rec[GPC_MAX_PYRAMID_LEVELS];
  const int32_t* d_cnt[GPC_MAX_PYRAMID_LEVELS];
  const uint8_t *a = d_a, *b = d_b;
  for (int l = 0; l < levels; ++l) {
    if (l) {
      uint8_t* na = (uint8_t*)c->py_img.p + img_at[l];
      uint8_t* nb = CORR ? nullptr : na + pad16((size_t)ws[l] * hs[l] * nimg);
      CHK(pyr_down(c, a, ws[l - 1], hs[l - 1], nimg, na));
      if (!CORR) CHK(pyr_down(c, b, ws[l - 1], hs[l - 1], nimg, nb));
      a = na;
      b = nb;
    }
    void* rec = (uint8_t*)c->py_rec.p + rec_at[l];
    int32_t* cnt = (int32_t*)c->py_cnt.p + (size_t)l * npairs;
    CHK(match(l, a, b, rec, caps[l], cnt));
    d_rec[l] = rec;
    d_cnt[l] = cnt;
  }
  return pyr_merge<CORR>(c, d_rec, caps, d_cnt, W, H, npairs, levels, d_out, cap, d_counts, d_level_counts);
}
}

int gpc_hip_pyramid_batch_device(gpc_hip_ctx* c, const uint8_t* d_rawL, const uint8_t* d_rawR, int W, int H, int npairs, int levels,
                                 const gpc_settings* s, gpc_support* d_out, int cap_per_pair, int32_t* d_counts,
                                 int32_t* d_level_counts, int32_t* d_ncand) {
  if (!c || !d_rawL || !d_rawR || !d_out || !d_counts || !d_level_counts || npairs <= 0 || cap_per_pair <= 0) return GPC_E_INVALID;
  return pyr_match<false>(c, d_rawL, d_rawR, W, H, npairs, levels, s, d_out, cap_per_pair, d_counts, d_level_counts, d_ncand);
}

int gpc_hip_pyramid_sequence_device(gpc_hip_ctx* c, const uint8_t* d_frames, int W, int H, int nframes, int levels,
                                    const gpc_settings* s, gpc_correspondence* d_out, int cap_per_pair, int32_t* d_counts,
                                    int32_t* d_level_counts, int32_t* d_ncand) {
  if (!c || !d_frames || !d_out || !d_counts || !d_level_counts || nframes < 2 || cap_per_pair <= 0) return GPC_E_INVALID;
  return pyr_match<true>(c, d_frames, nullptr, W, H, nframes - 1, levels, s, d_out, cap_per_pair, d_counts, d_level_counts,
                         d_ncand);
}

extern "C++" {
template <bool CORR>
static int pyr_host(gpc_hip_ctx* c, const uint8_t* a, const uint8_t* b, int W, int H, int npairs, int levels, const gpc_settings* s,
                    void* out, int cap, int32_t* counts, int32_t* level_counts, int32_t* ncand) {
  int32_t ws[GPC_MAX_PYRAMID_LEVELS], hs[GPC_MAX_PYRAMID_LEVELS];
  CHK(pyr_usable(c, s, W, H, levels, ws, hs));
  CHK(host_call_begin(c));
  const size_t n = (size_t)W * H, esz = sizeof(gpc::PyRec<CORR>);
  const int seq = CORR ? 1 : 0;
  const int most = CORR ? (c->seq_frames > 1 && c->seq_frames < 16 ? c->seq_frames : 16) - 1 : 16;
  const int K = npairs < most ? npairs : most;
  const size_t ncs = CORR ? (size_t)K + 1 : 2 * (size_t)K;
  const size_t total_ncs = CORR ? (size_t)npairs + 1 : 2 * (size_t)npairs;
  Stage st(c);
  const size_t r_a = st.in(n * (K + seq)), r_b = st.in(CORR ? 0 : n * K), r_out = st.out(esz * (size_t)cap * K);
  const size_t r_cnt = st.out(sizeof(int32_t) * (size_t)K), r_lc = st.out(sizeof(int32_t) * (size_t)levels * K);
  const size_t r_nc = st.out(sizeof(int32_t) * levels * ncs);
  CHK(st.alloc(sizeof(int32_t) * ((size_t)K + (size_t)levels * K + levels * ncs)));
  int status = GPC_OK;
  for (int p0 = 0; p0 < npairs; p0 += K) {
    const int pc = npairs - p0 < K ? npairs - p0 : K;
    const size_t cs = CORR ? (size_t)pc + 1 : 2 * (size_t)pc;
    CHK(st.up(r_a, a + n * p0, n * (pc + seq)));
    if (!CORR) CHK(st.up(r_b, b + n * p0, n * pc));
    CHK(pyr_match<CORR>(c, st.p(r_a), CORR ? nullptr : st.p(r_b), W, H, pc, levels, s, st.p(r_out), cap, (int32_t*)st.p(r_cnt),
                        (int32_t*)st.p(r_lc), (int32_t*)st.p(r_nc)));
    int32_t *h_n = c->h_cnt, *h_lc = h_n + K, *h_nc = h_lc + (size_t)levels * K;
    CHK(st.down(h_n, r_cnt, sizeof(int32_t) * (size_t)pc));
    CHK(st.down(h_lc, r_lc, sizeof(int32_t) * (size_t)levels * pc));
    CHK(st.down(h_nc, r_nc, sizeof(int32_t) * levels * cs));
    CHK(st.wait());
    for (int t = 0; t < pc; ++t) {
      const size_t w = (size_t)valid_records(h_n[t], cap), q = (size_t)(p0 + t);
      if (h_n[t] > cap) status = GPC_E_CAPACITY;
      if (w) CHK(st.down((uint8_t*)out + esz * q * cap, r_out + esz * (size_t)t * cap, esz * w));
      counts[q] = h_n[t];
      for (int l = 0; l < levels; ++l) level_counts[(size_t)l * npairs + q] = h_lc[(size_t)l * pc + t];
    }
    if (ncand)
      for (int l = 0; l < levels; ++l)
        memcpy(ncand + l * total_ncs + (CORR ? (size_t)p0 : 2 * (size_t)p0), h_nc + l * cs, sizeof(int32_t) * cs);
    CHK(st.wait());
  }
  CHK(check_join_err(c));
  return status;
}
}

int gpc_hip_pyramid_batch(gpc_hip_ctx* c, const uint8_t* rawL, const uint8_t* rawR, int W, int H, int npairs, int levels,
                          const gpc_settings* s, gpc_support* out, int cap_per_pair, int32_t* counts, int32_t* level_counts,
                          int32_t* ncand) {
  if (!c || !rawL || !rawR || !out || !counts || !level_counts || npairs <= 0 || cap_per_pair <= 0) return GPC_E_INVALID;
  return pyr_host<false>(c, rawL, rawR, W, H, npairs, levels, s, out, cap_per_pair, counts, level_counts, ncand);
}

int gpc_hip_pyramid_sequence(gpc_hip_ctx* c, const uint8_t* frames, int W, int H, int nframes, int levels, const gpc_settings* s,
                             gpc_correspondence* out, int cap_per_pair, int32_t* counts, int32_t* level_counts, int32_t* ncand) {
  if (!c || !frames || !out || !counts || !level_counts || nframes < 2 || cap_per_pair <= 0) return GPC_E_INVALID;
  return pyr_host<true>(c, frames, nullptr, W, H, nframes - 1, levels, s, out, cap_per_pair, counts, level_counts, ncand);
}

int gpc_hip_match_batch_device_packed(gpc_hip_ctx* c, const uint8_t* d_rawL, const uint8_t* d_rawR, int W, int H,
                                      int npairs, const gpc_settings* s, uint32_t* d_packed, int cap_per_pair,
                                      int32_t* d_rows, int32_t* d_counts, int32_t* d_ncand) {
  if (!c || !d_rawL || !d_rawR || !d_packed || !d_rows || !d_counts || npairs <= 0 || cap_per_pair <= 0) return GPC_E_INVALID;
  CHK(check_settings(s));
  if (!s->epipolar_mode || s->use_hashtable) return GPC_E_UNSUPPORTED;
  if (c->ngroups > 1) return GPC_E_UNSUPPORTED;
  CHK(check_dims(W, H));
  CHK(forest_matches(c, W, H));
  HIPCHK(c, hipSetDevice(c->device));
  const size_t n = (size_t)W * H;
  CHK(ensure(c, c->codes, sizeof(uint32_t) * n * 2 * npairs));
  CHK(run_preprocess(c, d_rawL, d_rawR, W, H, npairs, 2, s->gradient_threshold, true));
  CHK(run_hash(c, (const uint8_t*)c->smooth.p, (const uint8_t*)c->grad.p, nullptr, W, H, 2 * npairs, false,
               (uint32_t*)c->codes.p));
  const PackedOut po = {d_rows, (long)cap_per_pair, (long)H};
  CHK(run_match(c, W, H, npairs, s, 2, (const uint8_t*)c->grad.p, d_packed, cap_per_pair, d_counts, d_ncand, &po));
  return GPC_OK;
}

int gpc_hip_expand_packed(const uint32_t* packed, const int32_t* rows, int H, int n, gpc_support* out) {
  if (!packed || !rows || !out || H < 2 * GPC_R || n < 0) return GPC_E_INVALID;
  expand_rows(packed, rows, GPC_R, H - GPC_R, 0, n, out);
  return GPC_OK;
}

struct PackedHost {
  uint32_t* packed;
  int32_t* rows;
};
static int match_batch_packed(gpc_hip_ctx* c, const uint8_t* rawL, const uint8_t* rawR, int W, int H, int npairs,
                              const gpc_settings* s, gpc_support* out, int cap, int32_t* counts, int32_t* ncand,
                              const PackedHost* ph = nullptr);

static int match_batch_direct(gpc_hip_ctx* c, const uint8_t* rawL, const uint8_t* rawR, int W, int H, int npairs,
                              const gpc_settings* s, gpc_support* d_out_host, int cap, int32_t* counts, int32_t* ncand) {
  const size_t n = (size_t)W * H;
  CHK(ensure(c, c->raw, 2 * n * npairs));
  CHK(ensure(c, c->codes, sizeof(uint32_t) * n * 2 * npairs));
  CHK(pinned_counts(c, npairs));
  int32_t* d_cnt = nullptr;
  HIPCHK(c, hipHostGetDevicePointer((void**)&d_cnt, c->h_cnt, 0));
  uint8_t* d_l = (uint8_t*)c->raw.p;
  uint8_t* d_r = d_l + n * npairs;
  const void* vL = c->upload_mode ? device_view_of_host(rawL) : nullptr;
  const void* vR = vL ? device_view_of_host(rawR) : nullptr;
  const bool aligned = (((uintptr_t)vL | (uintptr_t)vR | (uintptr_t)d_l | (uintptr_t)d_r) & 15u) == 0 && (n * npairs) % 16 == 0 &&
                       n * npairs / 16 < (1ull << 31);
  if (vL && vR && aligned && c->upload_mode == 2) {
    d_l = (uint8_t*)vL;
    d_r = (uint8_t*)vR;
  } else if (vL && vR && aligned) {
    const unsigned n16 = (unsigned)(n * npairs / 16);
    hipLaunchKernelGGL(gpc::k_upload2, dim3((n16 + 255) / 256, 2), dim3(256), 0, c->stream, (const uint4*)vL, (const uint4*)vR,
                       (uint4*)d_l, (uint4*)d_r, n16);
    HIPCHK(c, hipGetLastError());
  } else {
    uint8_t* d_arena = nullptr;
    const size_t side = pad16(n * npairs);
    CHK(xfer_reserve(c, 2 * side, &d_arena));
    memcpy(c->h_xfer, rawL, n * npairs);
    memcpy(c->h_xfer + side, rawR, n * npairs);
    const unsigned n16 = (unsigned)(side / 16);
    CHK(ensure(c, c->raw, 2 * side));
    d_l = (uint8_t*)c->raw.p;
    d_r = d_l + side;
    hipLaunchKernelGGL(gpc::k_upload2, dim3((n16 + 255) / 256, 2), dim3(256), 0, c->stream, (const uint4*)d_arena,
                       (const uint4*)(d_arena + side), (uint4*)d_l, (uint4*)d_r, n16);
    HIPCHK(c, hipGetLastError());
  }
  CHK(run_preprocess(c, d_l, d_r, W, H, npairs, 2, s->gradient_threshold, true));
  CHK(run_hash(c, (const uint8_t*)c->smooth.p, (const uint8_t*)c->grad.p, nullptr, W, H, 2 * npairs, false, (uint32_t*)c->codes.p));
  CHK(run_match(c, W, H, npairs, s, 0, (const uint8_t*)c->grad.p, d_out_host, cap, d_cnt, d_cnt + npairs));
  HIPCHK(c, hipStreamSynchronize(c->stream));
  CHK(check_join_err(c));
  int status = GPC_OK;
  for (int p = 0; p < npairs; ++p) {
    counts[p] = c->h_cnt[p];
    if (counts[p] > cap) status = GPC_E_CAPACITY;
    if (ncand) {
      ncand[2 * p] = c->h_cnt[npairs + 2 * p];
      ncand[2 * p + 1] = c->h_cnt[npairs + 2 * p + 1];
    }
  }
  return status;
}

int gpc_hip_fed_calls(const gpc_hip_ctx* c) { return c ? c->fed_calls : 0; }

int gpc_hip_match_pair_begin(gpc_hip_ctx* c, const uint8_t* rawL, const uint8_t* rawR, int W, int H, const gpc_settings* s);

int gpc_hip_match_batch(gpc_hip_ctx* c, const uint8_t* rawL, const uint8_t* rawR, int W, int H, int npairs,
                        const gpc_settings* s, gpc_support* out, int cap, int32_t* counts, int32_t* ncand) {
  if (c && c->ngroups > 1) return GPC_E_UNSUPPORTED;
  if (c && npairs == 1 && rawL && rawR && out && counts && cap > 0 && s && !device_view_of_host(out)) {
    CHK(gpc_hip_match_pair_begin(c, rawL, rawR, W, H, s));
    int n = 0, nl = 0, nr = 0;
    const int st1 = match_fetch(c, out, cap, &n, &nl, &nr);
    c->pend.active = false;
    counts[0] = n;
    if (ncand) { ncand[0] = nl; ncand[1] = nr; }
    return st1;
  }
  const int st = on_gpu_node(c, npairs, [&] { return match_batch_packed(c, rawL, rawR, W, H, npairs, s, out, cap, counts, ncand); });
  if (c && st != GPC_OK && st != GPC_E_CAPACITY && st != GPC_E_INVALID) {
    c->pool.wait_all();
    if (c->s_in) {
      (void)hipStreamSynchronize(c->s_in);
      (void)hipStreamSynchronize(c->s_out);
      (void)hipStreamSynchronize(c->s_cnt);
    }
    if (c->s_aux) (void)hipStreamSynchronize(c->s_aux);
    (void)hipStreamSynchronize(c->stream);
  }
  return st;
}

static int match_batch_packed(gpc_hip_ctx* c, const uint8_t* rawL, const uint8_t* rawR, int W, int H, int npairs,
                              const gpc_settings* s, gpc_support* out, int cap, int32_t* counts, int32_t* ncand,
                              const PackedHost* ph) {
  if (!c || !rawL || !rawR || (!out && !ph) || !counts || npairs <= 0 || cap <= 0) return GPC_E_INVALID;
  if (ph && (!ph->packed || !ph->rows)) return GPC_E_INVALID;
  const double t_entry = host_ms();
  c->stage_ms[0] = c->stage_ms[1] = c->stage_ms[2] = c->stage_ms[3] = 0.f;
  CHK(check_settings(s));
  if (!s->epipolar_mode || s->use_hashtable) {
    if (ph) return GPC_E_UNSUPPORTED;
    return match_batch_unpacked(c, rawL, rawR, W, H, npairs, s, out, cap, counts, ncand);
  }
  CHK(check_dims(W, H));
  CHK(forest_matches(c, W, H));
  HIPCHK(c, hipSetDevice(c->device));
  if (!ph && npairs <= c->direct_max && (uint64_t)cap * sizeof(gpc_support) < (1ull << 32))
    if (void* dv = device_view_of_host(out))
      return match_batch_direct(c, rawL, rawR, W, H, npairs, s, (gpc_support*)dv, cap, counts, ncand);
  const size_t n = (size_t)W * H;
  int chunk = npairs < 4 ? npairs : (npairs / 8 < 1 ? 1 : (npairs / 8 > 16 ? 16 : npairs / 8));
  if (c->chunk_pairs > 0) chunk = c->chunk_pairs < npairs ? c->chunk_pairs : npairs;
  std::vector<int> c_start, c_size;
  {
    int rem = npairs, at = 0;
    auto put = [&](int m) {
      if (m <= 0) return;
      c_start.push_back(at);
      c_size.push_back(m);
      at += m;
      rem -= m;
    };
    const bool shaped = !c->flat_chunks && chunk >= 16 && npairs >= 4 * chunk;
    if (shaped) {
      put(chunk / 4);
      put(chunk - chunk / 4);
    }
    while (rem > chunk) put(chunk);
    if (shaped && rem >= 4) {
      const int r = rem;
      put(r / 2);
      put(r / 4);
      put(r - r / 2 - r / 4);
    } else {
      put(rem);
    }
  }
  const int nch = (int)c_size.size();
  const size_t rec = 4;
  const size_t hpad = ((size_t)H + 3) & ~(size_t)3;
  const size_t cb = 4 * hpad * chunk + ((rec * (size_t)cap * chunk + 15) & ~(size_t)15) + 16;
  CHK(ensure(c, c->raw, 2 * 2 * n * chunk));
  CHK(ensure(c, c->packed, 3 * cb + sizeof(int32_t) * 3 * chunk));
  CHK(ensure(c, c->counts, sizeof(int32_t) * npairs));
// ... 913 lines not shown
```

opengpc_amd/csrc/k_hash.h:

```cpp
#pragma once
#include "gpc_device.h"

namespace gpc {

#ifdef GPC_STAMPS
__device__ unsigned long long g_ht_stamps[16];
__device__ unsigned long long g_ht_wg[3 * 8192];
#define HT_STAMP(i)                                                                         \
  do {                                                                                      \
    unsigned long long t_;                                                                  \
    __builtin_amdgcn_sched_barrier(0);                                                      \
    asm volatile("s_memtime %0\n\ts_waitcnt lgkmcnt(0)" : "=s"(t_)::"memory");              \
    __builtin_amdgcn_sched_barrier(0);                                                      \
    ht_acc[i] += t_ - ht_t0;                                                                \
    ht_t0 = t_;                                                                             \
  } while (0)
#define HT_STAMP_FLUSH()                                                                    \
  if (threadIdx.x == 0) {  \
    unsigned long long rt2_;                                                                  \
    asm volatile("s_memrealtime %0\n\ts_waitcnt lgkmcnt(0)" : "=s"(rt2_)::"memory");         \
    atomicMax(&g_ht_stamps[8], (1ull << 62) - ht_rt0);                                        \
    atomicMax(&g_ht_stamps[9], ht_rt0);                                                       \
    atomicMax(&g_ht_stamps[10], rt2_);                                                        \
    const unsigned fb_ = blockIdx.x + gridDim.x * (blockIdx.y + gridDim.y * blockIdx.z);      \
// ... 71 lines not shown
}

typedef unsigned short gpc_ushort2 __attribute__((ext_vector_type(2)));
__device__ __forceinline__ uint32_t uaddsat_x4(uint32_t x, uint32_t t_hi) {
  const uint32_t xe = x << 8;
  gpc_ushort2 t, e, o;
  __builtin_memcpy(&t, &t_hi, 4);
  __builtin_memcpy(&e, &xe, 4);
  __builtin_memcpy(&o, &x, 4);
  e = __builtin_elementwise_add_sat(e, t);
  o = __builtin_elementwise_add_sat(o, t);
  uint32_t re, ro;
  __builtin_memcpy(&re, &e, 4);
  __builtin_memcpy(&ro, &o, 4);
  return __builtin_amdgcn_perm(ro, re, 0x07030501u);
}

template <bool TAU, bool NAIVE, int RPW>
__device__ __forceinline__ void fern_test(const uint8_t* __restrict__ tile, int lanebase, int packed, int tau,
                                          uint32_t (&plane)[RPW]) {
  const uint32_t* pa = reinterpret_cast<const uint32_t*>(tile + lanebase) + (int)(int16_t)(packed & 0xFFFF);
  const uint32_t* pb = reinterpret_cast<const uint32_t*>(tile + lanebase) + (packed >> 16);
#pragma unroll
  for (int r = 0; r < RPW; ++r) {
    uint32_t a = pa[r * (HT_STRIDE / 4)];
    uint32_t b = pb[r * (HT_STRIDE / 4)];
    uint32_t ge;
    if (TAU && NAIVE) {
      if (tau >= 1) {
        const uint32_t c = uaddsat_x4(a, (uint32_t)min(tau - 1, 255) * 0x01000100u);
        ge = ~swar_ge(b, c);
      } else {
        ge = swar_ge(a, uaddsat_x4(b, (uint32_t)min(-tau, 255) * 0x01000100u));
      }
    } else {
      if (TAU) b = subs_epi8x4(b, (uint32_t)(tau & 0xFF) * 0x01000100u);
      ge = swar_ge(a, b);
    }
    plane[r] = __builtin_amdgcn_bitop3_b32(ge, plane[r] >> 1, SW_H, 0xE4);
  }
}

#ifndef HT_PIPE
#define HT_PIPE 1
#endif
template <bool TAU, bool NAIVE, int RPW, int N, bool M128 = true>
__device__ __forceinline__ void fern_group(const uint8_t* __restrict__ tile, int lanebase,
                                           const GpcForestDev* __restrict__ fp, int t0, int cnt, uint32_t (&plane)[RPW]) {
#if HT_PIPE == 0
#pragma unroll
  for (int i = 0; i < N; ++i)
    if (i < cnt) fern_test<TAU, NAIVE, RPW>(tile, lanebase, fp->off[t0 + i], TAU ? fp->tau[t0 + i] : 0, plane);
#else
  constexpr int D = HT_PIPE + 1;
  uint32_t a[D][RPW], b[D][RPW];
  const uint32_t* base = reinterpret_cast<const uint32_t*>(tile + lanebase);
#ifndef HT_PACKED_OFFS
  uint32_t goff[2 * N];
#pragma unroll
  for (int i = 0; i < 2 * N; ++i) goff[i] = fp->boff[2 * t0 + i];
  uint32_t gk[N];
  if (TAU && !NAIVE) {
#pragma unroll
    for (int i = 0; i < N; ++i) gk[i] = (uint32_t)fp->tauk[t0 + i];
  }
#endif
  auto load = [&](int i, int slot) {
#ifndef HT_PACKED_OFFS
    const uint32_t* pa = reinterpret_cast<const uint32_t*>(reinterpret_cast<const uint8_t*>(base) + goff[2 * i]);
    const uint32_t* pb = reinterpret_cast<const uint32_t*>(reinterpret_cast<const uint8_t*>(base) + goff[2 * i + 1]);
#else
    const int packed = fp->off[t0 + i];
    const uint32_t* pa = base + (int)(int16_t)(packed & 0xFFFF);
    const uint32_t* pb = base + (packed >> 16);
#endif
#pragma unroll
    for (int r = 0; r < RPW; ++r) {
      a[slot][r] = pa[r * (HT_STRIDE / 4)];
      b[slot][r] = pb[r * (HT_STRIDE / 4)];
    }
  };
#pragma unroll
  for (int i = 0; i < HT_PIPE && i < N; ++i)
    if (i < cnt) load(i, i % D);
#pragma unroll
  for (int i = 0; i < N; ++i) {
    if (i + HT_PIPE < N && i + HT_PIPE < cnt) load(i + HT_PIPE, (i + HT_PIPE) % D);
    __builtin_amdgcn_sched_barrier(0);
    if (i < cnt) {
#ifndef HT_PACKED_OFFS
      const uint32_t k = (TAU && !NAIVE) ? gk[i] : 0u;
#else
      const uint32_t k = (TAU && !NAIVE) ? (uint32_t)fp->tauk[t0 + i] : 0u;
#endif
      const int tau = (TAU && NAIVE) ? fp->tau[t0 + i] : 0;
      if (TAU && !NAIVE && k != 0u) {
        {
#pragma unroll
          for (int r = 0; r < RPW; ++r) {
            const uint32_t gt = __builtin_amdgcn_lerp(a[i % D][r], subs_epi8x4_not<M128>(b[i % D][r], k), 0u);
            plane[r] = i == 0 ? ~gt : __builtin_amdgcn_bitop3_b32(gt, plane[r] >> 1, SW_H, 0x4E);
          }
        }
      } else {
#pragma unroll
        for (int r = 0; r < RPW; ++r) {
          uint32_t av = a[i % D][r], bv = b[i % D][r];
          uint32_t ge;
          if (TAU && NAIVE) {
            if (tau >= 1) {
              const uint32_t c = uaddsat_x4(av, (uint32_t)min(tau - 1, 255) * 0x01000100u);
              ge = ~swar_ge(bv, c);
            } else {
              ge = swar_ge(av, uaddsat_x4(bv, (uint32_t)min(-tau, 255) * 0x01000100u));
            }
          } else {
            ge = swar_ge(av, bv);
          }
          plane[r] = i == 0 ? ge : __builtin_amdgcn_bitop3_b32(ge, plane[r] >> 1, SW_H, 0xE4);
        }
      }
    }
    __builtin_amdgcn_sched_barrier(0);
  }
#endif
}

#ifndef HT_NO_SETPRIO
#define HT_PRIO_STEP(l) ht_set_prio(min((l), prio_cap))
#else
#define HT_PRIO_STEP(l) do { } while (0)
#endif
__device__ __forceinline__ void ht_set_prio(int lvl) {
  if (lvl >= 3) __builtin_amdgcn_s_setprio(3);
  else if (lvl == 2) __builtin_amdgcn_s_setprio(2);
  else if (lvl == 1) __builtin_amdgcn_s_setprio(1);
  else __builtin_amdgcn_s_setprio(0);
}

__device__ __forceinline__ uint32_t swar_nonzero(uint32_t x) { return (((x & SW_M) + SW_M) | x) & SW_H; }

#ifdef HT_WAVES_PER_EU
#define HT_OCC __attribute__((amdgpu_waves_per_eu(HT_WAVES_PER_EU, HT_WAVES_PER_EU)))
#else
#define HT_OCC
#endif
template <bool TAU, bool DENSE, bool NAIVE, bool GBITS = false, int TY = HT_Y>
__global__ __launch_bounds__(HT_THREADS) HT_OCC void k_hash(const uint8_t* __restrict__ smooth,
                                              const uint8_t* __restrict__ grad,
                                              const uint8_t* __restrict__ candmap,
                                              uint32_t* __restrict__ codes, int W, int H,
                                              const GpcForestDev* __restrict__ fp, int32_t* __restrict__ img_stats,
                                              int tpw, int last_round_from) {
#define HT_GROUPS 0
#include "k_hash_body.h"
#undef HT_GROUPS
}

__device__ __forceinline__ uint32_t ht_inv_cor(uint32_t cor3, uint32_t m3, int T) {
  uint32_t t = cor3 & m3;
  t |= t >> 16;
  t |= t >> 8;
  const int lowbits = T <= 8 ? T : (T - 1 < 24 ? T - 1 : 24);
  return ((t & 0x7Fu) << 24) | ((1u << lowbits) - 1u);
}

template <bool TAU, bool DENSE, bool NAIVE, bool GBITS = false, int TY = HT_Y>
__global__ __launch_bounds__(HT_THREADS) HT_OCC void k_hash_groups(const uint8_t* __restrict__ smooth,
                                              const uint8_t* __restrict__ grad,
                                              const uint8_t* __restrict__ candmap,
                                              uint32_t* __restrict__ codes, int W, int H,
                                              const GpcForestDev* __restrict__ fp_groups, int32_t* __restrict__ img_stats,
                                              int tpw, int last_round_from, int ngroups, int gstep) {
#define HT_GROUPS 1
#include "k_hash_body.h"
#undef HT_GROUPS
}

__global__ void k_scatter_mask(const int32_t* __restrict__ mask, int n_mask, uint8_t* __restrict__ candmap,
                               int W, int H) {
  const int i = blockIdx.x * blockDim.x + threadIdx.x;
  if (i >= n_mask) return;
  const int k = mask[i];
  if (k < 0 || k >= W * H) return;
  const int x = k % W, y = k / W;
  if (x >= GPC_R && x < W - GPC_R && y >= GPC_R && y < H - GPC_R) candmap[k] = 1;
}

}
```

opengpc_amd/csrc/k_hash_body.h:

```cpp
  static_assert(TY % (HT_THREADS / 64) == 0, "a wave owns TY / 8 rows of the tile");
  constexpr int RPW = TY / (HT_THREADS / 64);
  constexpr int T_ROWS = TY + 2 * GPC_R, T_COPY = T_ROWS * HT_STRIDE;
  __shared__ __attribute__((aligned(16))) uint8_t tile[4 * T_COPY];
  __shared__ int s_cnt, s_last, s_or;
#if HT_GROUPS
  __shared__ int s_gor[GPC_MAX_GROUPS];
  const GpcForestDev* __restrict__ fp = fp_groups;
#endif

  unsigned bx = blockIdx.x, by = blockIdx.y, bz = blockIdx.z;
#ifndef HT_NO_XCD_REMAP
  {
    const unsigned nwg = gridDim.x * gridDim.y * gridDim.z;
    if ((nwg & 7u) == 0u) {
      const unsigned flat = blockIdx.x + gridDim.x * (blockIdx.y + gridDim.y * blockIdx.z);
      const unsigned logical = (flat & 7u) * (nwg >> 3) + (flat >> 3);
      bx = logical % gridDim.x;
      by = (logical / gridDim.x) % gridDim.y;
      bz = logical / (gridDim.x * gridDim.y);
    }
  }
#endif
  const int img = bz;
  const long n = (long)W * H;
  const uint8_t* sm = smooth + (long)img * n;
  static_assert(!GBITS || (!DENSE && !NAIVE), "the bit image exists in the batched SSE pipelines only");
  const uint8_t* gr = grad + (long)img * (GBITS ? n / 8 : n);
  const uint8_t* cm = (!GBITS && candmap) ? candmap + (long)img * n : nullptr;
#if !HT_GROUPS
  uint32_t* out = codes + (long)img * n;
#endif
  const int tx0 = bx * HT_X;
  const int tid = threadIdx.x;
  const int wave = tid >> 6, lane = tid & 63;
  const int x0 = tx0 + 4 * lane;

  if (tid == 0) { s_cnt = 0; s_last = -1; s_or = 0; }
#if HT_GROUPS
  if (tid < GPC_MAX_GROUPS) s_gor[tid] = 0;
#endif

  uint32_t xmask = 0u;
#pragma unroll
  for (int j = 0; j < 4; ++j)
    if (x0 + j >= GPC_R && x0 + j < W - GPC_R) xmask |= 0x80u << (8 * j);

  constexpr int QPR = HT_STRIDE / 16;
  constexpr int NCHUNK = T_ROWS * QPR;
  constexpr int CPT = (NCHUNK + HT_THREADS - 1) / HT_THREADS;
  int crow[CPT], cnxt[CPT], cdst[CPT];
  uint32_t cflag[CPT];
#pragma unroll
  for (int i = 0; i < CPT; ++i) {
    const int c = tid + i * HT_THREADS;
    const int r = c / QPR, q = c - r * QPR;
    crow[i] = c < NCHUNK ? r * W + q * 16 - HT_APRON + tx0 : HT_FAR;
    cnxt[i] = (c < NCHUNK && q + 1 < QPR) ? crow[i] + 16 : HT_FAR;
    cdst[i] = r * HT_STRIDE + q * 16;
    cflag[i] = (c < NCHUNK ? 1u : 0u) | (q + 1 < QPR ? 2u : 0u);
  }
  uint4 pv[CPT];
  uint32_t pn[CPT];
  uint32_t pg[RPW];
  const uint32_t nbytes = (uint32_t)n;
  const __amdgpu_buffer_rsrc_t rs_sm = __builtin_amdgcn_make_buffer_rsrc(const_cast<uint8_t*>(sm), 0, (int)nbytes, 0x00020000);
  const __amdgpu_buffer_rsrc_t rs_gr = __builtin_amdgcn_make_buffer_rsrc(const_cast<uint8_t*>(gr), 0, (int)(GBITS ? nbytes / 8u : nbytes), 0x00020000);
  const uint32_t gcol = x0 < W ? (GBITS ? (uint32_t)(x0 & ~15) >> 3 : (uint32_t)x0) : (uint32_t)HT_FAR;
  auto fetch = [&](int ty0) {
#pragma unroll
    for (int r = 0; r < RPW; ++r) {
      const int y = ty0 + wave * RPW + r;
      if (GBITS)
        pg[r] = (uint32_t)__builtin_amdgcn_raw_buffer_load_b16(rs_gr, ((uint32_t)(y * W) >> 3) + gcol, 0, 0);
      else
        pg[r] = __builtin_amdgcn_raw_buffer_load_b32(rs_gr, (uint32_t)(y * W) + gcol, 0, 0);
    }
    const int base = (ty0 - GPC_R) * W;
#pragma unroll
    for (int i = 0; i < CPT; ++i) {
      const uint32_t k = (uint32_t)(base + crow[i]);
      typedef uint32_t u32x4 __attribute__((ext_vector_type(4)));
      const u32x4 v = __builtin_amdgcn_raw_buffer_load_b128(rs_sm, k, 0, 0);
      pn[i] = __builtin_amdgcn_raw_buffer_load_b32(rs_sm, (uint32_t)(base + cnxt[i]), 0, 0);
      pv[i] = make_uint4(v.x, v.y, v.z, v.w);
    }
  };
  auto stage = [&]() {
#pragma unroll
    for (int i = 0; i < CPT; ++i) {
      if (cflag[i] & 1u) {
        uint8_t* dst = tile + cdst[i];
        const uint4 v = pv[i];
        *reinterpret_cast<uint4*>(dst) = v;
#pragma unroll
        for (int sft = 1; sft < 4; ++sft) {
          uint4 w;
          w.x = __builtin_amdgcn_alignbyte(v.y, v.x, sft);
          w.y = __builtin_amdgcn_alignbyte(v.z, v.y, sft);
          w.z = __builtin_amdgcn_alignbyte(v.w, v.z, sft);
          w.w = __builtin_amdgcn_alignbyte(pn[i], v.w, sft);
          *reinterpret_cast<uint4*>(dst + sft * T_COPY) = w;
        }
      }
    }
  };

  constexpr bool INV = !DENSE && !NAIVE;
  constexpr int CBIT = GBITS ? 0 : 7;
  const int tile0 = by * tpw;
  const int ntiles = (H - 2 * GPC_R + TY - 1) / TY;
  const bool last_round = (int)(blockIdx.x + gridDim.x * (blockIdx.y + gridDim.y * blockIdx.z)) >= last_round_from;
  HT_STAMP_INIT();
  fetch(GPC_R + tile0 * TY);
  int cnt = 0, last = -1;
  uint32_t cor = 0u;
  uint32_t cor3 = 0u;
  const int T = fp->num_tests;
  const bool m128 = TAU && !NAIVE && fp->tau_m128 != 0;
  int lanebase = (wave * RPW + GPC_R) * HT_STRIDE + 4 * lane + HT_APRON;
  asm volatile("" : "+v"(lanebase));
  const int n3 = max(1, min(T, 32) - 25);
  const uint32_t m3 = 0x01010101u * ((1u << n3) - 1u);
  const uint32_t m8 = (x0 & 4) ? 0x01010101u : 0x01010100u;
#pragma unroll 1
  for (int tt = 0; tt < tpw && tile0 + tt < ntiles; ++tt) {
  const int ty0 = GPC_R + (tile0 + tt) * TY;
#ifndef HT_NO_SETPRIO
  int prio_cap = 3;
  if (last_round) {
    const int left = min(tpw - tt, ntiles - tile0 - tt);
    prio_cap = left >= 6 ? 3 : left >= 4 ? 2 : left >= 2 ? 1 : 0;
  }
  ht_set_prio(prio_cap);
#endif
  if (tt) __syncthreads();
  HT_STAMP(0);
  stage();
  uint32_t gq[RPW];
#pragma unroll
  for (int r = 0; r < RPW; ++r) gq[r] = pg[r];
  __syncthreads();
  HT_STAMP(1);
  if (tt + 1 < tpw && tile0 + tt + 1 < ntiles) fetch(ty0 + TY);
  HT_STAMP(2);

  const int yw = ty0 + wave * RPW;

  uint32_t cand8[RPW];
  bool rowdo[RPW];
  bool any = false;
  if (GBITS) {
#pragma unroll
    for (int r = 0; r < RPW; ++r) {
      const int y = yw + r;
      const uint32_t g4 = gq[r];
      const uint32_t nib = __builtin_amdgcn_ubfe(g4, (uint32_t)(x0 & 15), 4u);
      const uint32_t cb = __umul24(nib, 0x204081u) & (xmask >> 7) & (y < H - GPC_R ? ~0u : 0u);
      cand8[r] = cb;
      rowdo[r] = (y < H - 15) & (g4 != 0u);
      any = any | ((cb != 0u) & rowdo[r]);
    }
  } else
#pragma unroll
  for (int r = 0; r < RPW; ++r) {
    const int y = yw + r;
    const uint32_t g4 = gq[r];
    uint32_t c4 = g4;
    if (cm) c4 = (x0 < W && y < H) ? *reinterpret_cast<const uint32_t*>(cm + (uint32_t)(y * W + x0)) : 0u;
    uint32_t cb;
    if (GBITS && !cm) {
      const uint32_t nib = (g4 >> (x0 & 15)) & 0xFu;
      cb = (y < H - GPC_R) ? ((nib * 0x10204080u) & SW_H & xmask) : 0u;
    } else {
      cb = (y < H - GPC_R) ? (swar_nonzero(c4) & xmask) : 0u;
    }
    uint32_t gany = g4;
    if (!NAIVE && !GBITS) {
      gany |= (uint32_t)__builtin_amdgcn_mov_dpp((int)gany, 0xB1, 0xF, 0xF, true);
      gany |= (uint32_t)__builtin_amdgcn_mov_dpp((int)gany, 0x4E, 0xF, 0xF, true);
    }
    const bool rows_ok = y < (NAIVE ? H - GPC_R : H - 15);
    cand8[r] = cb;
    rowdo[r] = (x0 < W) && rows_ok && (NAIVE || gany != 0u);
    any = any || ((DENSE && !NAIVE) ? rowdo[r] : (cb != 0u && rowdo[r]));
  }

#if HT_GROUPS
#pragma unroll 1
  for (int g = 0; g < ngroups; ++g) {
  const GpcForestDev* __restrict__ fp = fp_groups + g;
  const int T = fp->num_tests;
  const bool m128 = TAU && !NAIVE && fp->tau_m128 != 0;
  const int n3 = max(1, min(T, 32) - 25);
  const uint32_t m3 = 0x01010101u * ((1u << n3) - 1u);
  uint32_t* out = codes + (long)((img >> 1) * 2 * ngroups + (img & 1) + g * gstep) * n;
  uint32_t cor = 0u, cor3 = 0u;
#ifndef HT_NO_SETPRIO
  if (g) ht_set_prio(prio_cap);
#endif
#endif
  uint32_t code[RPW][4];
#pragma unroll
  for (int r = 0; r < RPW; ++r)
#pragma unroll
    for (int j = 0; j < 4; ++j) code[r][j] = INV ? ~0u : 0u;
  HT_STAMP(3);

#ifdef HT_EXP_NOCOMPUTE
  if (W < 0) {
#else
  if (__ballot(any)) {
#endif
    uint32_t p0[RPW], p1[RPW], p2[RPW], p3[RPW], p8[RPW];
#pragma unroll
    for (int r = 0; r < RPW; ++r) p0[r] = p1[r] = p2[r] = p3[r] = p8[r] = ~0u;
    if (NAIVE) {
      if (T > 0) fern_group<TAU, true, RPW, 8>(tile, lanebase, fp, 0, 8, p0);
      HT_PRIO_STEP(2);
      if (T > 8) fern_group<TAU, true, RPW, 8>(tile, lanebase, fp, 8, 8, p1);
      HT_PRIO_STEP(1);
      if (T > 16) fern_group<TAU, true, RPW, 8>(tile, lanebase, fp, 16, 8, p2);
      HT_PRIO_STEP(0);
      if (T > 24) fern_group<TAU, true, RPW, 8>(tile, lanebase, fp, 24, 8, p3);
    } else if (TAU && m128) {
      if (T > 0) fern_group<TAU, false, RPW, 8, true>(tile, lanebase, fp, 0, 8, p0);
      if (T > 8) fern_group<TAU, false, RPW, 1, true>(tile, lanebase, fp, 8, 1, p8);
      HT_PRIO_STEP(2);
      if (T > 9) fern_group<TAU, false, RPW, 8, true>(tile, lanebase, fp, 9, 8, p1);
      HT_PRIO_STEP(1);
      if (T > 17) fern_group<TAU, false, RPW, 8, true>(tile, lanebase, fp, 17, 8, p2);
      HT_PRIO_STEP(0);
      if (T > 25) fern_group<TAU, false, RPW, 7, true>(tile, lanebase, fp, 25, min(T, 32) - 25, p3);
    } else {
      if (T > 0) fern_group<TAU, false, RPW, 8, false>(tile, lanebase, fp, 0, 8, p0);
      if (T > 8) fern_group<TAU, false, RPW, 1, false>(tile, lanebase, fp, 8, 1, p8);
      HT_PRIO_STEP(2);
      if (T > 9) fern_group<TAU, false, RPW, 8, false>(tile, lanebase, fp, 9, 8, p1);
      HT_PRIO_STEP(1);
      if (T > 17) fern_group<TAU, false, RPW, 8, false>(tile, lanebase, fp, 17, 8, p2);
      HT_PRIO_STEP(0);
      if (T > 25) fern_group<TAU, false, RPW, 7, false>(tile, lanebase, fp, 25, min(T, 32) - 25, p3);
    }
#pragma unroll
    for (int r = 0; r < RPW; ++r) {
      const uint32_t q0 = INV ? (p0[r] & ((p8[r] >> 7) | ~m8)) : (NAIVE ? ~p0[r] : (~p0[r] | ((~p8[r] >> 7) & m8)));
      const uint32_t q1 = INV ? p1[r] : ~p1[r];
      const uint32_t q2 = INV ? p2[r] : ~p2[r];
      const uint32_t q3 = INV ? ((p3[r] >> (8 - n3)) | ~m3) : (NAIVE ? ~p3[r] : ((~p3[r] >> (8 - n3)) & m3));
      if (INV) cor3 = __builtin_amdgcn_bitop3_b32(q3, rowdo[r] ? ~0u : 0u, cor3, 0xAE);
      const uint32_t lo01 = __builtin_amdgcn_perm(q1, q0, 0x05010400u);
      const uint32_t hi01 = __builtin_amdgcn_perm(q1, q0, 0x07030602u);
      const uint32_t lo23 = __builtin_amdgcn_perm(q3, q2, 0x05010400u);
      const uint32_t hi23 = __builtin_amdgcn_perm(q3, q2, 0x07030602u);
      code[r][0] = __builtin_amdgcn_perm(lo23, lo01, 0x05040100u);
      code[r][1] = __builtin_amdgcn_perm(lo23, lo01, 0x07060302u);
      code[r][2] = __builtin_amdgcn_perm(hi23, hi01, 0x05040100u);
      code[r][3] = __builtin_amdgcn_perm(hi23, hi01, 0x07060302u);
    }
  }

  HT_STAMP(4);
#pragma unroll
  for (int r = 0; r < RPW; ++r) {
    const int y = yw + r;
    if ((x0 < W) && (y < H)) {
      uint4 o;
      uint32_t* op = reinterpret_cast<uint32_t*>(&o);
      if (DENSE) {
#pragma unroll
        for (int j = 0; j < 4; ++j) {
          const uint32_t c = rowdo[r] ? code[r][j] : 0u;
          cor |= c;
          const bool is_cand = (cand8[r] >> (8 * j + 7)) & 1u;
          op[j] = (NAIVE && !is_cand) ? 0u : c;
        }
      } else {
        const uint32_t dom = rowdo[r] ? ~0u : 0u;
#pragma unroll
        for (int j = 0; j < 4; ++j) {
          const uint32_t cm4 = (uint32_t)__builtin_amdgcn_sbfe((int)cand8[r], 8 * j + CBIT, 1);
          if (INV) {
            op[j] = __builtin_amdgcn_bitop3_b32(code[r][j], dom, cm4, 0x5D);
          } else {
            cor |= code[r][j] & dom;
            op[j] = __builtin_amdgcn_bitop3_b32(code[r][j], dom, cm4, 0xD5);
          }
        }
      }
#if defined(HT_EXP_NOSTORE)
      if (o.x == 0x12345678u && W < 0) *reinterpret_cast<uint4*>(out + (uint32_t)(y * W + x0)) = o;
#elif defined(HT_EXP_HALFSTORE)
      if ((lane & 1) == 0) *reinterpret_cast<uint4*>(out + (uint32_t)(y * W + x0)) = o;
#else
      *reinterpret_cast<uint4*>(out + (uint32_t)(y * W + x0)) = o;
#endif
    }
#if HT_GROUPS
    if (g == 0 && cand8[r]) { cnt += __popc(cand8[r]); last = y; }
#else
    if (cand8[r]) { cnt += __popc(cand8[r]); last = y; }
#endif
  }
#if HT_GROUPS
  if (!DENSE) {
    uint32_t t = INV ? ht_inv_cor(cor3, m3, T) : cor;
    for (int o = 32; o > 0; o >>= 1) t |= (uint32_t)__shfl_xor((int)t, o);
    if (lane == 0 && t) atomicOr(&s_gor[g], (int)t);
  }
  }
#endif
  HT_STAMP(5);
  }
  HT_STAMP_FLUSH();
#if !HT_GROUPS
  if (INV) {
    uint32_t t = cor3 & m3;
    t |= t >> 16;
    t |= t >> 8;
    const int lowbits = T <= 8 ? T : (T - 1 < 24 ? T - 1 : 24);
    cor = ((t & 0x7Fu) << 24) | ((1u << lowbits) - 1u);
  }
#endif
  if (!DENSE) {
    for (int o = 32; o > 0; o >>= 1) {
      cnt += __shfl_xor(cnt, o);
      last = max(last, __shfl_xor(last, o));
      cor |= (uint32_t)__shfl_xor((int)cor, o);
    }
    if (lane == 0 && cnt) { atomicAdd(&s_cnt, cnt); atomicMax(&s_last, last); atomicOr(&s_or, (int)cor); }
    __syncthreads();
#if HT_GROUPS
    if (tid < ngroups && s_cnt) {
      const int v = (img >> 1) * 2 * ngroups + (img & 1) + tid * gstep;
      atomicAdd(&img_stats[v * GPC_STAT_STRIDE + GPC_STAT_NCAND], s_cnt);
      atomicMax(&img_stats[v * GPC_STAT_STRIDE + GPC_STAT_LASTROW], s_last);
      atomicOr(&img_stats[v * GPC_STAT_STRIDE + GPC_STAT_CODEOR], s_gor[tid]);
    }
#else
    if (tid == 0 && s_cnt) {
      atomicAdd(&img_stats[img * GPC_STAT_STRIDE + GPC_STAT_NCAND], s_cnt);
      atomicMax(&img_stats[img * GPC_STAT_STRIDE + GPC_STAT_LASTROW], s_last);
      atomicOr(&img_stats[img * GPC_STAT_STRIDE + GPC_STAT_CODEOR], s_or);
    }
#endif
  }
```

opengpc_amd/csrc/k_rowjoin_fused.h:

```cpp
#pragma once
#include <cstddef>

#include "k_rowjoin.h"

namespace gpc {

#define RJ_SHARDS 64
#define RJ_TICKET_STRIDE 32
#define RJ_ST_AGG 1u
#define RJ_ST_PREFIX 2u
#define RJ_SPIN_LIMIT (1 << 18)

struct RjfArgs {
  const uint32_t* codes;
  const uint8_t* cand;
  const int32_t* img_stats;
  uint32_t* tickets;
  unsigned long long* status;
  int32_t* err;
  void* out;
  int32_t* counts;
  int32_t* ncand;
  int32_t* rows_out;
  long packed_stride, rows_stride;
// ... 56 lines not shown
    base += (uint32_t)__builtin_amdgcn_readlane((int)c, 63);
    return first_p < 64 ? 1 : 0;
  };
  int r = window(g);
  if (r == 0) pos -= 64;
  while (r != 1) {
    if (r < 0) {
#ifdef RJ_DBG_COUNT
      if (lane == 0) atomicAdd(err + 2, 1);
#endif
      if (++spin > RJ_SPIN_LIMIT) {
        if (lane == 0) __hip_atomic_store(err, (int32_t)epoch, __ATOMIC_RELAXED, __HIP_MEMORY_SCOPE_SYSTEM);
        break;
      }
      __builtin_amdgcn_s_sleep(2);
    }
    unsigned long long gw[RJ_LB_WINDOWS];
#pragma unroll
    for (int k = 0; k < RJ_LB_WINDOWS; ++k) gw[k] = rjf_lookback_ask(st - (t - 1 - (pos - 64 * k)), pos - 64 * k + 1, lane, epoch);
#pragma unroll
    for (int k = 0; k < RJ_LB_WINDOWS; ++k) {
      r = window(gw[k]);
      if (r != 0) break;
      pos -= 64;
    }
  }
  return base;
}

template <int NT>
__device__ __forceinline__ void rjf_emit_row(const uint32_t* __restrict__ words, uint32_t cnt, uint32_t base, int pair, int y, int tid) {
#ifdef RJ_DBG_NOEMIT
  return;
#endif
  RjfK* a = rjf_args();
  const int mode = a->mode, cap = a->cap;
  if (mode == 0) {
    struct __attribute__((packed, aligned(4))) Rec3 { uint32_t x, y, d; };
    Rec3* o = reinterpret_cast<Rec3*>(a->out) + (long)pair * cap;
    for (uint32_t i = tid; i < cnt; i += NT) {
      const uint32_t w = words[i], p = base + i;
      const int xl = (int)(w & 0xFFFFu), xr = (int)(w >> 16);
      if (p < (uint32_t)cap) o[p] = Rec3{(uint32_t)xl, (uint32_t)y, __float_as_uint((float)(xl - xr))};
    }
  } else if (mode == 2) {
    uint32_t* o = reinterpret_cast<uint32_t*>(a->out) + pair * a->packed_stride;
    for (uint32_t i = tid; i < cnt; i += NT) {
      const uint32_t p = base + i;
      if (p < (uint32_t)cap) o[p] = words[i];
    }
    if (tid == 0) a->rows_out[pair * a->rows_stride + y] = (int32_t)cnt;
  } else {
    int4* o = reinterpret_cast<int4*>(a->out) + (long)pair * cap;
    for (uint32_t i = tid; i < cnt; i += NT) {
      const uint32_t w = words[i], p = base + i;
      if (p < (uint32_t)cap) o[p] = make_int4((int)(w & 0xFFFFu), y, (int)(w >> 16), y);
    }
  }
}

__device__ __forceinline__ void rjf_finish_pair(int pair, uint32_t total) {
  RjfK* a = rjf_args();
  a->counts[pair] = (int32_t)total;
  int32_t* nc = a->ncand;
  if (nc) {
    const int32_t* st = a->img_stats;
    nc[pair * 2 + 0] = st[(pair * 2 + 0) * GPC_STAT_STRIDE + GPC_STAT_NCAND];
    nc[pair * 2 + 1] = st[(pair * 2 + 1) * GPC_STAT_STRIDE + GPC_STAT_NCAND];
  }
}

#ifdef RJF_CHECK_EXEC
#define RJF_EXEC_ALL "s_mov_b64 exec, -1\n\t"
#define RJF_ASSERT_EXEC_ALL() do { if (__builtin_amdgcn_read_exec() != ~0ull) __builtin_trap(); } while (0)
#else
#define RJF_EXEC_ALL "s_mov_b64 exec, -1"
#define RJF_ASSERT_EXEC_ALL() do { } while (0)
#endif

__device__ __forceinline__ uint32_t rjf_walk(uint32_t keys_lds, uint32_t s0, uint32_t cnt, uint32_t cj) {
  uint32_t rank = s0, addr, k;
  asm volatile(
      "v_cmpx_lt_u32_e32 vcc, 1, %[cnt]\n\t"
      "s_cbranch_execz 2f\n\t"
      "v_lshl_add_u32 %[addr], %[s0], 2, %[base]\n"
      "1:\n\t"
      "ds_read_b32 %[k], %[addr]\n\t"
      "v_add_u32_e32 %[addr], 4, %[addr]\n\t"
      "v_add_u32_e32 %[cnt], -1, %[cnt]\n\t"
      "s_waitcnt lgkmcnt(0)\n\t"
      "v_cmp_lt_u32_e32 vcc, %[k], %[cj]\n\t"
      "v_addc_co_u32_e32 %[rank], vcc, 0, %[rank], vcc\n\t"
      "v_cmpx_ne_u32_e32 vcc, 0, %[cnt]\n\t"
      "s_cbranch_execnz 1b\n"
      "2:\n\t"
      RJF_EXEC_ALL
      : [rank] "+v"(rank), [cnt] "+v"(cnt), [addr] "=&v"(addr), [k] "=&v"(k)
      : [s0] "v"(s0), [cj] "v"(cj), [base] "s"(keys_lds)
      : "vcc", "memory");
  return rank;
}

__device__ __forceinline__ void rjf_insert_chain(uint32_t keys_lds, uint32_t& cur, uint32_t& o, uint32_t h, uint32_t smask) {
  uint32_t addr;
  asm volatile(
      "v_cmpx_ne_u32_e32 vcc, 0, %[cur]\n\t"
      "v_cmpx_ne_u32_e32 vcc, 0, %[o]\n\t"
      "v_cmpx_ne_u32_e32 vcc, %[o], %[cur]\n\t"
      "s_cbranch_execz 2f\n"
      "1:\n\t"
      "v_min_u32_e32 %[cur], %[o], %[cur]\n\t"
      "v_add_u32_e32 %[h], 1, %[h]\n\t"
      "v_and_b32_e32 %[h], %[smask], %[h]\n\t"
      "v_lshl_add_u32 %[addr], %[h], 2, %[base]\n\t"
      "ds_max_rtn_u32 %[o], %[addr], %[cur]\n\t"
      "s_waitcnt lgkmcnt(0)\n\t"
      "v_cmpx_ne_u32_e32 vcc, 0, %[o]\n\t"
      "v_cmpx_ne_u32_e32 vcc, %[o], %[cur]\n\t"
      "s_cbranch_execnz 1b\n"
      "2:\n\t"
      RJF_EXEC_ALL
      : [cur] "+v"(cur), [o] "+v"(o), [h] "+v"(h), [addr] "=&v"(addr)
      : [smask] "s"(smask), [base] "s"(keys_lds)
      : "vcc", "memory");
}

__device__ __forceinline__ uint32_t rjf_find_chain(uint32_t keys_lds, uint32_t k, uint32_t& kk, uint32_t h, uint32_t smask) {
  uint32_t addr;
  asm volatile(
      "v_cmpx_gt_u32_e32 vcc, %[kk], %[k]\n\t"
      "s_cbranch_execz 2f\n"
      "1:\n\t"
      "v_add_u32_e32 %[h], 1, %[h]\n\t"
      "v_and_b32_e32 %[h], %[smask], %[h]\n\t"
      "v_lshl_add_u32 %[addr], %[h], 2, %[base]\n\t"
      "ds_read_b32 %[kk], %[addr]\n\t"
      "s_waitcnt lgkmcnt(0)\n\t"
      "v_cmpx_gt_u32_e32 vcc, %[kk], %[k]\n\t"
      "s_cbranch_execnz 1b\n"
      "2:\n\t"
      RJF_EXEC_ALL
      : [kk] "+v"(kk), [h] "+v"(h), [addr] "=&v"(addr)
      : [k] "v"(k), [smask] "s"(smask), [base] "s"(keys_lds)
      : "vcc", "memory");
  return h;
}

__device__ __forceinline__ uint32_t rjf_home(uint32_t k, uint32_t idx, int shift, uint32_t smask, bool wide) {
  if (wide) return k ? rj_hash(k, shift) : (idx & smask);
  const uint32_t none = (uint32_t)((int32_t)(k - 1u) >> 31);
  return rj_hash(k, shift) | (idx & smask & none);
}

constexpr int rjf_log2(int v) {
  int l = 0;
  while ((1 << l) < v) ++l;
  return l;
}

#define RJF_LDS_BYTES(NB) ((size_t)6 * pow2_at_least(2 * (NB)) + (size_t)4 * (NB) + (size_t)4 * ((NB) - 24))
#ifndef RJF_PRIO_PAT
#define RJF_PRIO_PAT 0x0123333
#endif
#ifndef RJF_NO_PRIO
#define RJF_PRIO(ph) __builtin_amdgcn_s_setprio((RJF_PRIO_PAT >> (4 * (6 - (ph)))) & 3)
#else
#define RJF_PRIO(ph) do { } while (0)
#endif
#ifdef GPC_WGLIFE
__device__ unsigned long long g_rjf_wg[3 * 4096];
#endif
template <int SPT, int NT, bool WIDE>
__global__ __launch_bounds__(NT) __attribute__((amdgpu_waves_per_eu(8, 8))) void k_row_join_fused(RjfArgs ka) {
#ifdef GPC_WGLIFE
  unsigned long long wl_t0;
  unsigned wl_rows = 0u;
  asm volatile("s_memrealtime %0\n\ts_waitcnt lgkmcnt(0)" : "=s"(wl_t0)::"memory");
#endif
  static_assert(SPT <= 4 && NT * SPT <= 4096, "16-bit flag words hold 12 bits of x");
  static_assert(NT >= 128, "the second wave draws the tickets");
  constexpr int NB = NT * SPT, S = 1 << rjf_log2(2 * NB);
  constexpr uint32_t smask = (uint32_t)S - 1u;
  constexpr int hshift = 32 - rjf_log2(S);
  constexpr uint32_t F_LDUP = 0x2000u, F_RSEEN = 0x4000u, F_RDUP = 0x8000u, F_XMASK = 0x0FFFu;
  extern __shared__ __attribute__((aligned(16))) uint32_t rjf_lds[];
  __shared__ uint32_t s_max_key;
  __shared__ int s_tail_cnt;
  __shared__ unsigned s_tail_minx;
  __shared__ int s_sp_l, s_sp_r;
  __shared__ unsigned s_sp_minx;
  __shared__ uint32_t s_w[NT / 64];
  __shared__ uint32_t s_ticket, s_base;
  __shared__ uint32_t s_cnt;
  uint32_t* const t_key = rjf_lds;
  uint32_t* const t_w = rjf_lds + S;
  uint32_t* const r_cnt = rjf_lds + S + S / 2;
  uint32_t* const d_words = r_cnt + NB;
  uint32_t* const r_key = t_w;
  static_assert((sizeof(uint32_t) * (12 + NT / 64)) % 16 == 0, "the dynamic block follows the static variables without padding");
  const uint32_t keys_lds = __builtin_amdgcn_groupstaticsize();
  const uint32_t rkey_lds = keys_lds + 4u * (uint32_t)S;

  int f_shard, f_ps, f_sh;
  uint32_t f_magic, f_end, f_g;
  {
    RjfK* a = rjf_args();
    f_shard = (int)(blockIdx.x % (unsigned)a->nshards);
    const int hi = f_shard < a->n_hi ? 0 : 1;
    f_ps = a->ps[hi];
    f_magic = a->ps_magic[hi];
    f_sh = a->ps_sh[hi];
    f_end = (uint32_t)f_ps * (uint32_t)(a->H - 2 * GPC_R);
    if (threadIdx.x == 0) {
      uint32_t opaque0;
      asm volatile("v_mov_b32 %0, 0" : "=v"(opaque0));
      s_ticket = __hip_atomic_fetch_add(a->tickets + f_shard * RJ_TICKET_STRIDE + opaque0, 1u, __ATOMIC_RELAXED, __HIP_MEMORY_SCOPE_AGENT);
    }
    __syncthreads();
    f_g = (uint32_t)__builtin_amdgcn_readfirstlane((int)s_ticket);
  }
  int d_pair = 0, d_t = -1;
  uint32_t d_cnt = 0u;
  unsigned long long d_g0 = 0ull;
  uint32_t f_nxt = 0u;

  uint32_t ncl[SPT], ncr[SPT];
  auto row_of = [&](uint32_t g) -> const uint32_t* {
    const uint32_t q = (f_ps == 1) ? g : (__umulhi(g, f_magic) >> f_sh);
    const int W = ka.W, H = ka.H;
    const int pair = f_shard + ka.nshards * (int)(g - q * (uint32_t)f_ps);
    const long ro = ((long)(pair * 2) * H + (GPC_R + (int)q)) * W;
    return ka.codes + ro;
  };
  auto issue_loads = [&](const uint32_t* rl, uint32_t (&cl)[SPT], uint32_t (&cr)[SPT]) {
    const uint32_t* rr_ = rl + (long)ka.H * ka.W;
    uint32_t lo = threadIdx.x * 4u;
    RJF_OPAQUE_V(lo);
#pragma unroll
    for (int j = 0; j < SPT; ++j) {
      cl[j] = *reinterpret_cast<const uint32_t*>(reinterpret_cast<const char*>(rl) + lo + (uint32_t)(j * NT * 4));
      cr[j] = *reinterpret_cast<const uint32_t*>(reinterpret_cast<const char*>(rr_) + lo + (uint32_t)(j * NT * 4));
    }
  };
  if (f_g < f_end) issue_loads(row_of(f_g), ncl, ncr);

#pragma unroll 1
  while (f_g < f_end) {
    int tid = threadIdx.x;
    RJF_OPAQUE_V(tid);
    const int lane = tid & 63;
    const uint32_t q = (f_ps == 1) ? f_g : (__umulhi(f_g, f_magic) >> f_sh);
    const int f_t = (int)q, y = GPC_R + f_t;
    int pair, W;
    uint32_t nspl = 0u, nspr = 0u;
    bool tail_row;
    int csh;
    {
      W = ka.W;
      const int H = ka.H;
      pair = f_shard + ka.nshards * (int)(f_g - q * (uint32_t)f_ps);
      const long ro = ((long)(pair * 2) * H + y) * W;
      typedef const int32_t __attribute__((address_space(4))) kint;
      kint* st = (kint*)ka.img_stats;
      tail_row = (y == st[(pair * 2 + 1) * GPC_STAT_STRIDE + GPC_STAT_LASTROW]);
      const uint32_t span = (uint32_t)st[(pair * 2) * GPC_STAT_STRIDE + GPC_STAT_CODEOR];
      csh = (span ? 32 - __builtin_clz(span) : 0) - (rjf_log2(NB + 1) - 1);
      if (csh < 0) csh = 0;
      if (WIDE) {
        const uint8_t* cand = ka.cand;
#pragma unroll
        for (int j = 0; j < SPT; ++j) {
          const int x = j * NT + tid;
          const bool inm = x >= GPC_R && x < W - GPC_R;
          if (inm && ncl[j] == RJ_EMPTY && cand[ro + x]) nspl |= 1u << j;
          if (inm && ncr[j] == RJ_EMPTY && cand[ro + (long)H * W + x]) nspr |= 1u << j;
        }
      }
    }
    RJ_STAMP_INIT();
    RJF_PRIO(0);
    uint32_t kl[SPT], kr[SPT];
#pragma unroll
    for (int j = 0; j < SPT; ++j) {
      const uint32_t inm = (uint32_t)((j * NT + tid - W) >> 31);
      kl[j] = (ncl[j] + 1u) & inm;
      kr[j] = (ncr[j] + 1u) & inm;
#ifdef RJ_DBG_EMPTY
      kl[j] = kr[j] = 0u * (ncl[j] + ncr[j]);
#endif
    }
    const uint32_t spl = WIDE ? nspl : 0u, spr = WIDE ? nspr : 0u;
    {
      uint32_t z0;
      asm volatile("v_mov_b32 %0, 0" : "=v"(z0));
      const uint4 zero = make_uint4(z0, z0, z0, z0);
      uint4* zk = reinterpret_cast<uint4*>(t_key);
      constexpr int NZK = S / 4, NZC = NB / 4;
#pragma unroll
      for (int i = 0; i < (NZK + NT - 1) / NT; ++i)
        if (NZK % NT == 0 || tid + i * NT < NZK) zk[tid + i * NT] = zero;
      uint4* zc = reinterpret_cast<uint4*>(r_cnt);
#pragma unroll
      for (int i = 0; i < (NZC + NT - 1) / NT; ++i)
        if (NZC % NT == 0 || tid + i * NT < NZC) zc[tid + i * NT] = zero;
      if (tid == 0) {
        s_max_key = z0;
        s_tail_cnt = (int)z0;
        s_tail_minx = ~z0;
        s_cnt = z0;
        if (WIDE) {
          s_sp_l = (int)z0;
          s_sp_r = (int)z0;
          s_sp_minx = ~z0;
        }
      }
    }
    __syncthreads();
    RJ_STAMP(0);
    RJF_PRIO(1);

    uint32_t h0l[SPT];
    bool ldup[SPT];
    uint32_t carried[SPT];
#pragma unroll
    for (int j = 0; j < SPT; ++j) carried[j] = 0u;
    {
      uint32_t old[SPT];
#pragma unroll
      for (int j = 0; j < SPT; ++j) {
        h0l[j] = rjf_home(kl[j], (uint32_t)(j * NT + tid), hshift, smask, WIDE);
        old[j] = atomicMax(&t_key[h0l[j]], kl[j]);
      }
      {
        uint32_t z0;
        asm volatile("v_mov_b32 %0, 0" : "=v"(z0));
        uint4* zf = reinterpret_cast<uint4*>(t_w);
        constexpr int NZF = S / 2 / 4;
#pragma unroll
        for (int i = 0; i < (NZF + NT - 1) / NT; ++i)
          if (NZF % NT == 0 || tid + i * NT < NZF) zf[tid + i * NT] = make_uint4(z0, z0, z0, z0);
      }
#pragma unroll
      for (int j = 0; j < SPT; ++j) {
        uint32_t cur = kl[j], o = old[j];
        RJF_ASSERT_EXEC_ALL();
        rjf_insert_chain(keys_lds, cur, o, h0l[j], smask);
        const bool met = kl[j] && o == cur;
        ldup[j] = met && cur == kl[j];
        if (met && cur != kl[j]) carried[j] = cur;
      }
    }
    if (tail_row) {
      uint32_t max_k = 0;
#pragma unroll
      for (int j = 0; j < SPT; ++j) max_k = max(max_k, kr[j]);
      max_k = wave_max_u32(max_k);
      if (lane == 0 && max_k) atomicMax(&s_max_key, max_k);
    }
    if (WIDE) {
      if (__ballot(spl != 0u) | __ballot(spr != 0u)) {
        if (spl) atomicAdd(&s_sp_l, __popc(spl));
        if (spr) {
          atomicAdd(&s_sp_r, __popc(spr));
          atomicMin(&s_sp_minx, (unsigned)((__ffs((int)spr) - 1) * NT + tid));
        }
      }
    }
    if (tid == 64) {
      uint32_t opaque0;
      asm volatile("v_mov_b32 %0, 0" : "=v"(opaque0));
      f_nxt = __hip_atomic_fetch_add(rjf_args()->tickets + f_shard * RJ_TICKET_STRIDE + opaque0, 1u, __ATOMIC_RELAXED, __HIP_MEMORY_SCOPE_AGENT);
    }
    __syncthreads();
    RJ_STAMP(1);
    RJF_PRIO(2);
    if (d_t >= 0 && tid < 64) {
      RjfK* a = rjf_args();
      d_g0 = rjf_lookback_ask(a->status + (long)d_pair * (ka.H - 2 * GPC_R) + d_t, d_t, lane, a->epoch);
    }

    uint32_t hl[SPT];
    {
      uint32_t h0r[SPT], f0l[SPT], f0r[SPT];
#pragma unroll
      for (int j = 0; j < SPT; ++j) {
        h0r[j] = rjf_home(kr[j], (uint32_t)(j * NT + tid), hshift, smask, WIDE);
        f0l[j] = t_key[h0l[j]];
        f0r[j] = t_key[h0r[j]];
      }
      uint32_t seen[SPT], mv[SPT];
      uint32_t ql[SPT], qr[SPT];
#pragma unroll
      for (int j = 0; j < SPT; ++j) {
        ql[j] = WIDE ? kl[j] : (kl[j] | (uint32_t)((int32_t)(kl[j] - 1u) >> 31));
        qr[j] = WIDE ? kr[j] : (kr[j] | (uint32_t)((int32_t)(kr[j] - 1u) >> 31));
      }
      {
#pragma unroll
        for (int j = 0; j < SPT; ++j) {
          uint32_t kk = WIDE ? (kl[j] ? f0l[j] : 0u) : f0l[j];
          RJF_ASSERT_EXEC_ALL();
          hl[j] = rjf_find_chain(keys_lds, ql[j], kk, h0l[j], smask);
        }
      }
#pragma unroll
      for (int j = 0; j < SPT; ++j)
        if (ldup[j]) atomicOr(&t_w[hl[j] >> 1], F_LDUP << ((hl[j] & 1u) << 4));
      {
        uint32_t anyc = 0u;
#pragma unroll
        for (int j = 0; j < SPT; ++j) anyc |= carried[j];
        if (__ballot(anyc != 0u)) {
#pragma unroll
          for (int j = 0; j < SPT; ++j) {
            const uint32_t hc0 = rj_hash(carried[j], hshift);
            uint32_t kk = carried[j] ? t_key[hc0] : 0u;
            RJF_ASSERT_EXEC_ALL();
            const uint32_t hc = rjf_find_chain(keys_lds, carried[j], kk, hc0, smask);
            if (carried[j]) atomicOr(&t_w[hc >> 1], F_LDUP << ((hc & 1u) << 4));
#ifdef RJ_DBG_COUNT
            if (carried[j]) atomicAdd(rjf_args()->err + 3, 1);
#endif
          }
        }
      }
      uint32_t hr[SPT];
#pragma unroll
      for (int j = 0; j < SPT; ++j) {
        uint32_t kk = WIDE ? (kr[j] ? f0r[j] : 0u) : f0r[j];
        RJF_ASSERT_EXEC_ALL();
        hr[j] = rjf_find_chain(keys_lds, qr[j], kk, h0r[j], smask);
        const bool hit = WIDE ? (kr[j] && kk == kr[j]) : (kk == qr[j]);
        mv[j] = (hit ? (F_RSEEN | (uint32_t)(j * NT + tid)) : 0u) << ((hr[j] & 1u) << 4);
      }
#pragma unroll
      for (int j = 0; j < SPT; ++j) seen[j] = atomicOr(&t_w[hr[j] >> 1], mv[j]);
#pragma unroll
      for (int j = 0; j < SPT; ++j) {
        const uint32_t again = seen[j] & mv[j] & (F_RSEEN | (F_RSEEN << 16));
        if (again) atomicOr(&t_w[hr[j] >> 1], again << 1);
      }
    }
    uint32_t tail_key = 0u;
    bool tail_sp = false;
    if (tail_row) {
      tail_sp = WIDE && s_sp_r > 0;
      tail_key = tail_sp ? 0u : s_max_key;
#pragma unroll
      for (int j = 0; j < SPT; ++j)
        if (kr[j] && kr[j] == tail_key) {
          atomicAdd(&s_tail_cnt, 1);
          atomicMin(&s_tail_minx, (unsigned)(j * NT + tid));
        }
    }
    __syncthreads();
    RJ_STAMP(2);
    RJF_PRIO(3);
    if (d_t >= 0 && tid < 64) {
      RjfK* a = rjf_args();
      unsigned long long* d_st = a->status + (long)d_pair * (ka.H - 2 * GPC_R) + d_t;
      const uint32_t ep = a->epoch;
      const uint32_t base = rjf_lookback(d_st, d_t, lane, ep, d_g0, a->err);
      if (lane == 0) {
        if (d_t > 0) __hip_atomic_store(d_st, rjf_granule(ep, RJ_ST_PREFIX, base + d_cnt), __ATOMIC_RELAXED, __HIP_MEMORY_SCOPE_AGENT);
        s_base = base;
      }
    }

    bool ok[SPT];
    uint32_t xr[SPT];
    uint32_t wc = 0u;
    const int disp_high = ka.disp_high, apply_filter = ka.apply_filter;
#ifndef RJF_OLD_DECIDE
    if (!WIDE && !tail_row) {
      uint32_t w[SPT];
#pragma unroll
      for (int j = 0; j < SPT; ++j) w[j] = reinterpret_cast<const uint16_t*>(t_w)[hl[j]];
#pragma unroll
      for (int j = 0; j < SPT; ++j) {
        xr[j] = w[j] & F_XMASK;
        uint32_t has = kl[j];
        asm volatile("" : "+v"(has));
        const bool hit = (has != 0u) & ((w[j] & (F_LDUP | F_RSEEN | F_RDUP)) == F_RSEEN);
        const bool near = (apply_filter == 0) | ((int)__usad((uint32_t)(j * NT + tid), xr[j], 0u) <= disp_high);
        const bool good = hit & near;
        wc += (uint32_t)__builtin_popcountll(__builtin_amdgcn_ballot_w64(good));
        ok[j] = good;
      }
    } else
#endif
    {
#pragma unroll
      for (int j = 0; j < SPT; ++j) {
        xr[j] = 0u;
        bool good = false;
        if (kl[j]) {
          const uint32_t w = reinterpret_cast<const uint16_t*>(t_w)[hl[j]];
          const bool tail = tail_row && kl[j] == tail_key;
          good = !(w & F_LDUP) && (tail ? (s_tail_cnt == 2) : ((w & (F_RSEEN | F_RDUP)) == F_RSEEN));
          xr[j] = tail ? s_tail_minx : (w & F_XMASK);
        } else if (WIDE && ((spl >> j) & 1u)) {
          good = (s_sp_l == 1) && (s_sp_r == (tail_sp ? 2 : 1));
          xr[j] = s_sp_minx;
        }
        if (good && apply_filter) good = abs((int)(j * NT + tid) - (int)xr[j]) <= disp_high;
        ok[j] = good;
        wc += (uint32_t)__popcll(__ballot(good));
      }
    }
    uint32_t rb[SPT], rs[SPT];
#pragma unroll
    for (int j = 0; j < SPT; ++j) {
      rb[j] = (kl[j] - 1u) >> csh;
      rs[j] = 0u;
      if (ok[j]) rs[j] = atomicAdd(&r_cnt[rb[j]], 1u);
    }
    if (lane == 0 && wc) atomicAdd(&s_cnt, wc);
    if (tid == 64) s_ticket = f_nxt;
    __syncthreads();
    RJ_STAMP(3);
    RJF_PRIO(4);
    const uint32_t f_cnt = (uint32_t)__builtin_amdgcn_readfirstlane((int)s_cnt);
    if (tid == 0) {
      RjfK* a = rjf_args();
      __hip_atomic_store(a->status + (long)pair * (ka.H - 2 * GPC_R) + f_t, rjf_granule(a->epoch, f_t == 0 ? RJ_ST_PREFIX : RJ_ST_AGG, f_cnt),
                         __ATOMIC_RELAXED, __HIP_MEMORY_SCOPE_AGENT);
    }
    const uint32_t f_gn = (uint32_t)__builtin_amdgcn_readfirstlane((int)s_ticket);

#pragma unroll
    for (int j = 0; j < SPT; ++j)
      if (ok[j]) rs[j] |= r_cnt[rb[j]] << 16;
    if (d_t >= 0) {
      const uint32_t base = s_base;
      rjf_emit_row<NT>(d_words, d_cnt, base, d_pair, GPC_R + d_t, tid);
      if (tid == 0 && d_t == ka.H - 2 * GPC_R - 1) rjf_finish_pair(d_pair, base + d_cnt);
    }
    RJ_STAMP(4);
    RJF_PRIO(5);
    block_exscan<SPT, NT, false>(r_cnt, s_w, tid);
#pragma unroll
    for (int j = 0; j < SPT; ++j)
      if (ok[j]) {
        rb[j] = r_cnt[rb[j]];
        if ((rs[j] >> 16) > 1u) r_key[rb[j] + (rs[j] & 0xFFFFu)] = kl[j] - 1u;
      }
    __syncthreads();
    RJ_STAMP(5);
    RJF_PRIO(6);
#pragma unroll
    for (int j = 0; j < SPT; ++j) {
      const bool m = ok[j];
      RJF_ASSERT_EXEC_ALL();
      const uint32_t rank = rjf_walk(rkey_lds, rb[j], rs[j] >> 16, kl[j] - 1u);
      if (m) d_words[rank] = (uint32_t)(j * NT + tid) | (xr[j] << 16);
    }
    d_pair = pair;
    d_t = f_t;
    d_cnt = f_cnt;
    f_g = f_gn;
    if (f_g < f_end) issue_loads(row_of(f_g), ncl, ncr);
#ifdef GPC_STAMPS
    asm volatile("s_waitcnt vmcnt(0)" ::: "memory");
#endif
    RJ_STAMP(6);
    RJ_STAMP_FLUSH();
#ifdef GPC_WGLIFE
    ++wl_rows;
#endif
  }

  {
    RjfK* a = rjf_args();
    const int nrows = a->H - 2 * GPC_R;
    const uint32_t f_last = f_end + (gridDim.x - (unsigned)f_shard + (unsigned)a->nshards - 1u) / (unsigned)a->nshards - 1u;
    if (threadIdx.x == 0 && f_g == f_last)
      __hip_atomic_store(a->tickets + f_shard * RJ_TICKET_STRIDE, 0u, __ATOMIC_RELAXED, __HIP_MEMORY_SCOPE_AGENT);
    if (d_t >= 0) {
      if (threadIdx.x < 64) {
        const int lane = threadIdx.x;
        unsigned long long* d_st = a->status + (long)d_pair * nrows + d_t;
        const uint32_t ep = a->epoch;
        const uint32_t base = rjf_lookback(d_st, d_t, lane, ep, rjf_lookback_ask(d_st, d_t, lane, ep), a->err);
        if (lane == 0) {
          if (d_t > 0) __hip_atomic_store(d_st, rjf_granule(ep, RJ_ST_PREFIX, base + d_cnt), __ATOMIC_RELAXED, __HIP_MEMORY_SCOPE_AGENT);
          s_base = base;
        }
      }
      __syncthreads();
      const uint32_t base = s_base;
      rjf_emit_row<NT>(d_words, d_cnt, base, d_pair, GPC_R + d_t, threadIdx.x);
      if (threadIdx.x == 0 && d_t == nrows - 1) rjf_finish_pair(d_pair, base + d_cnt);
    }
  }
#ifdef GPC_WGLIFE
  if (threadIdx.x == 0 && blockIdx.x < 4096u) {
    unsigned long long t1_;
    unsigned hw_, xcc_;
    asm volatile("s_memrealtime %0\n\ts_waitcnt lgkmcnt(0)" : "=s"(t1_)::"memory");
    asm volatile("s_getreg_b32 %0, hwreg(HW_REG_HW_ID)" : "=s"(hw_));
    asm volatile("s_getreg_b32 %0, hwreg(HW_REG_XCC_ID)" : "=s"(xcc_));
    g_rjf_wg[3 * blockIdx.x] = wl_t0;
    g_rjf_wg[3 * blockIdx.x + 1] = t1_;
    g_rjf_wg[3 * blockIdx.x + 2] = ((unsigned long long)wl_rows << 40) | ((unsigned long long)(xcc_ & 0xFu) << 32) | hw_;
  }
#endif
}

}
```

Measured before the change: 248,500 Mpix/s.

## Emit pre-keyed codes from hash kernel so fused row join skips key prep

Adds a keyed variant of the hash kernel that writes codes in a key format, with bit 31 tagging the no-code or invalid case and codes kept below 2^31. A matching keyed variant of the fused row-join kernel consumes these codes directly. The per-element +1, masking, home-slot and query computations become cheaper, and an exact-width form drops the bounds mask entirely. It is gated by a heuristic and an env var, and relies on non-wide codes that fit in 31 bits.

```diff
diff --git a/opengpc_amd/csrc/gpc_hip.hip b/opengpc_amd/csrc/gpc_hip.hip
--- a/opengpc_amd/csrc/gpc_hip.hip
+++ b/opengpc_amd/csrc/gpc_hip.hip
@@ -274,6 +274,8 @@
   int32_t* h_err = nullptr;
   int32_t* d_err = nullptr;
   int no_fuse = 0;
+  int no_keyed = 0;
+  int keyed_always = 0;
   int fuse_always = 0;
   int fuse_wgs = 0;
   int fuse_min_pairs = 1;
@@ -698,9 +700,11 @@
 }
 
 int run_hash(gpc_hip_ctx* c, const uint8_t* d_smooth, const uint8_t* d_grad, const uint8_t* d_cand,
-             int W, int H, int nimg, bool dense, uint32_t* d_codes, int groups = 0, int gstep = 2, int32_t* d_stats = nullptr) {
+             int W, int H, int nimg, bool dense, uint32_t* d_codes, int groups = 0, int gstep = 2, int32_t* d_stats = nullptr,
+             bool keyed = false) {
   if (!c->have_forest) return GPC_E_NO_FOREST;
   const bool gbits = c->grad_is_bits && d_grad == (const uint8_t*)c->grad.p && !dense && !c->naive && d_cand == nullptr;
+  if (keyed && (!gbits || groups > 0)) return GPC_E_INVALID;
   const int slots = 2 * (c->num_cus > 0 ? c->num_cus : 256);
   const int gx = (W + HT_X - 1) / HT_X;
   int ty = HT_Y;
@@ -769,12 +773,24 @@
     HIPCHK(c, hipGetLastError());
     return GPC_OK;
   }
+  if (keyed) snprintf(c->launch_name[KID_HASH], sizeof c->launch_name[0], "gpc::k_hash_keyed<%s, %d>", tau ? "true" : "false", ty);
+  else
   snprintf(c->launch_name[KID_HASH], sizeof c->launch_name[0], "gpc::k_hash<%s, %s, %s, %s, %d>", tau ? "true" : "false",
            dense ? "true" : "false", c->naive ? "true" : "false", gbits ? "true" : "false", ty);
 #define LAUNCH_HASH(TAU, DENSE, NAIVE)                                                                    \
   hipLaunchKernelGGL((gpc::k_hash<TAU, DENSE, NAIVE>), grid, dim3(HT_THREADS), 0, c->stream, d_smooth, d_grad, \
                      d_cand, d_codes, W, H, (const GpcForestDev*)c->forest_dev.p + (NAIVE ? 1 : 0), st, tpw, last_from)
-  if (gbits) {
+  if (keyed) {
+#define LAUNCH_HASH_KEYED(TAU, TY, FD)                                                                            \
+  hipLaunchKernelGGL((gpc::k_hash_keyed<TAU, TY>), grid, dim3(HT_THREADS), 0, c->stream, d_smooth, d_grad,        \
+                     d_cand, d_codes, W, H, (const GpcForestDev*)c->forest_dev.p + FD, st, tpw, last_from)
+    if (ty == HT_Y_TALL) {
+      if (tau) LAUNCH_HASH_KEYED(true, HT_Y_TALL, 2); else LAUNCH_HASH_KEYED(false, HT_Y_TALL, 2);
+    } else {
+      if (tau) LAUNCH_HASH_KEYED(true, HT_Y, 0); else LAUNCH_HASH_KEYED(false, HT_Y, 0);
+    }
+#undef LAUNCH_HASH_KEYED
+  } else if (gbits) {
 #define LAUNCH_HASH_BITS(TAU, TY, FD)                                                                                      \
   hipLaunchKernelGGL((gpc::k_hash<TAU, false, false, true, TY>), grid, dim3(HT_THREADS), 0, c->stream, d_smooth, d_grad, \
                      d_cand, d_codes, W, H, (const GpcForestDev*)c->forest_dev.p + FD, st, tpw, last_from)
@@ -884,9 +900,30 @@
   return GPC_OK;
 }
 
+bool join_fuses(const gpc_hip_ctx* c, int W, int H, int npairs, bool gapfree, bool seq, bool by_size = false) {
+  const JoinPlan jp = plan_join(c, W);
+  const size_t flds = RJF_LDS_BYTES(jp.nt * jp.spt);
+  bool fuse = !seq && !c->no_fuse && npairs >= c->fuse_min_pairs && jp.spt <= 4 && jp.nt * jp.spt <= 4096 &&
+              !gapfree && (long)npairs * (H - 2 * GPC_R) < (1l << 31) - 65536;
+  if (fuse && (by_size || !c->fuse_always)) {
+    const long lds_wgs = (long)(160 * 1024 / (flds + 64)), wave_wgs = 32 / (jp.nt / 64);
+    const long resident = (long)c->num_cus * (lds_wgs < wave_wgs ? lds_wgs : wave_wgs);
+    const long rows_total = (long)npairs * (H - 2 * GPC_R);
+    fuse = rows_total >= 4 * resident || (W >= 2048 && rows_total >= 3 * resident);
+  }
+  return fuse;
+}
+
+bool keyed_codes(const gpc_hip_ctx* c, int W, int H, int npairs, const gpc_settings* s) {
+  if (c->no_keyed || !s->epipolar_mode || s->use_hashtable || c->naive || c->ngroups > 1 || !c->grad_is_bits) return false;
+  return join_fuses(c, W, H, npairs, false, false) && (c->keyed_always || join_fuses(c, W, H, npairs, false, false, true));
+}
+
 int run_match(gpc_hip_ctx* c, int W, int H, int npairs, const gpc_settings* s, int mode, const uint8_t* d_cand,
-              void* d_out, int cap, int32_t* d_counts, int32_t* d_ncand, const PackedOut* po = nullptr, bool seq = false) {
+              void* d_out, int cap, int32_t* d_counts, int32_t* d_ncand, const PackedOut* po = nullptr, bool seq = false,
+              bool keyed = false) {
   const int apply_filter = (mode != 1);
+  if (keyed && (s->use_hashtable || !s->epipolar_mode || !join_fuses(c, W, H, npairs, po && po->totals, seq))) return GPC_E_INVALID;
   if (mode == 2 && (s->use_hashtable || !s->epipolar_mode || !po)) return GPC_E_UNSUPPORTED;
   if (seq && (mode == 2 || po)) return GPC_E_UNSUPPORTED;
   if (s->use_hashtable) return run_hashtable_match(c, W, H, npairs, s, mode, d_cand, d_out, cap, d_counts, d_ncand, seq);
@@ -898,14 +935,7 @@
     const JoinPlan jp = plan_join(c, W);
     if (jp.nt * jp.spt < W) return GPC_E_UNSUPPORTED;
     const size_t flds = RJF_LDS_BYTES(jp.nt * jp.spt);
-    bool fuse = !seq && !c->no_fuse && npairs >= c->fuse_min_pairs && jp.spt <= 4 && jp.nt * jp.spt <= 4096 &&
-                !(po && po->totals) && (long)npairs * (H - 2 * GPC_R) < (1l << 31) - 65536;
-    if (fuse && !c->fuse_always) {
-      const long lds_wgs = (long)(160 * 1024 / (flds + 64)), wave_wgs = 32 / (jp.nt / 64);
-      const long resident = (long)c->num_cus * (lds_wgs < wave_wgs ? lds_wgs : wave_wgs);
-      const long rows_total = (long)npairs * (H - 2 * GPC_R);
-      fuse = rows_total >= 4 * resident || (W >= 2048 && rows_total >= 3 * resident);
-    }
+    const bool fuse = join_fuses(c, W, H, npairs, po && po->totals, seq);
     if (fuse) {
       const int nrows = H - 2 * GPC_R;
       CHK(check_join_err(c));
@@ -935,12 +965,19 @@
       a.cap = cap;
       Timed t(c, KID_ROW_JOIN);
       const bool wide = wide_codes(c);
+      if (keyed && wide) return GPC_E_INVALID;
+      const bool exact = W == jp.nt * jp.spt;
+      if (keyed)
+        snprintf(c->launch_name[KID_ROW_JOIN], sizeof c->launch_name[0], "gpc::k_row_join_fused_keyed<%d, %d, %s>", jp.spt, jp.nt,
+                 exact ? "true" : "false");
+      else
       snprintf(c->launch_name[KID_ROW_JOIN], sizeof c->launch_name[0], "gpc::k_row_join_fused<%d, %d, %s>", jp.spt, jp.nt,
                wide ? "true" : "false");
       c->launch_name[KID_GATHER_ROWS][0] = 0;
-#define LAUNCH_RJF(SPT, NT, WIDE)                                                                               \
+#define LAUNCH_RJF(SPT, NT, WIDE) LAUNCH_RJF_K(k_row_join_fused, SPT, NT, WIDE)
+#define LAUNCH_RJF_K(K, SPT, NT, WIDE)                                                                          \
   do {                                                                                                          \
-    const void* fn_ = reinterpret_cast<const void*>(gpc::k_row_join_fused<SPT, NT, WIDE>);                      \
+    const void* fn_ = reinterpret_cast<const void*>(gpc::K<SPT, NT, WIDE>);                                     \
     int& per_cu = c->wgs_per_cu[std::make_pair(fn_, lds)];                                                      \
     if (per_cu == 0) {                                                                                          \
       if (lds > 48 * 1024) CHK(allow_dyn_lds(c, fn_, lds));                                                     \
@@ -962,9 +999,14 @@
       a.ps_magic[k_] = sp_.ps_magic[k_];                                                                        \
       a.ps_sh[k_] = sp_.ps_sh[k_];                                                                              \
     }                                                                                                           \
-    hipLaunchKernelGGL((gpc::k_row_join_fused<SPT, NT, WIDE>), dim3((unsigned)nwg), dim3(NT), lds, c->stream, a); \
+    hipLaunchKernelGGL((gpc::K<SPT, NT, WIDE>), dim3((unsigned)nwg), dim3(NT), lds, c->stream, a);              \
   } while (0)
-#define LAUNCH_RJF_W(SPT, NT) do { if (wide) LAUNCH_RJF(SPT, NT, true); else LAUNCH_RJF(SPT, NT, false); } while (0)
+#define LAUNCH_RJF_W(SPT, NT)                                                                                   \
+  do {                                                                                                          \
+    if (keyed) { if (exact) LAUNCH_RJF_K(k_row_join_fused_keyed, SPT, NT, true); else LAUNCH_RJF_K(k_row_join_fused_keyed, SPT, NT, false); } \
+    else if (wide) LAUNCH_RJF(SPT, NT, true);                                                                   \
+    else LAUNCH_RJF(SPT, NT, false);                                                                            \
+  } while (0)
 #define LAUNCH_RJF_S(NT)                      \
   switch (jp.spt) {                           \
     case 1: LAUNCH_RJF_W(1, NT); break;       \
@@ -976,6 +1018,7 @@
       else { LAUNCH_RJF_S(256) }
 #undef LAUNCH_RJF_S
 #undef LAUNCH_RJF_W
+#undef LAUNCH_RJF_K
 #undef LAUNCH_RJF
       HIPCHK(c, hipGetLastError());
       return GPC_OK;
@@ -1922,6 +1965,8 @@
   c->no_feeder = getenv("GPC_HIP_NO_FEEDER") != nullptr;
   c->no_pair_packed = getenv("GPC_HIP_NO_PAIR_PACKED") != nullptr;
   c->no_fuse = getenv("GPC_HIP_NO_FUSE") != nullptr;
+  c->no_keyed = getenv("GPC_HIP_NO_KEYED") != nullptr;
+  if (const char* e = getenv("GPC_HIP_KEYED")) c->keyed_always = atoi(e) ? 1 : 0;
   if (const char* e = getenv("GPC_HIP_HASH_TALL")) c->hash_tall = atoi(e) ? 1 : 0;
   if (const char* e = getenv("GPC_HIP_PRE_ROWS")) {
     const int v = atoi(e);
@@ -2754,9 +2799,11 @@
     lane.used = true;
     CHK(ensure(c, c->codes, sizeof(uint32_t) * n * 2 * npairs));
     CHK(run_preprocess(c, d_rawL, d_rawR, W, H, npairs, 2, s->gradient_threshold, true));
-    CHK(run_hash(c, (const uint8_t*)c->smooth.p, (const uint8_t*)c->grad.p, nullptr, W, H, 2 * npairs, false, (uint32_t*)c->codes.p));
+    const bool keyed = keyed_codes(c, W, H, npairs, s);
+    CHK(run_hash(c, (const uint8_t*)c->smooth.p, (const uint8_t*)c->grad.p, nullptr, W, H, 2 * npairs, false, (uint32_t*)c->codes.p,
+                 0, 2, nullptr, keyed));
     HIPCHK(c, hipEventRecord(lane.e_hash, c->stream));
-    CHK(run_match(c, W, H, npairs, s, 0, (const uint8_t*)c->grad.p, d_out, cap_per_pair, d_counts, d_ncand));
+    CHK(run_match(c, W, H, npairs, s, 0, (const uint8_t*)c->grad.p, d_out, cap_per_pair, d_counts, d_ncand, nullptr, false, keyed));
     HIPCHK(c, hipEventRecord(lane.e_join, c->stream));
     return GPC_OK;
   }
@@ -2765,10 +2812,11 @@
   if (c->dbg_wait_pre) HIPCHK(c, hipStreamWaitEvent(c->stream, c->dbg_wait_pre, 0));
   CHK(run_preprocess(c, d_rawL, d_rawR, W, H, npairs, 2, s->gradient_threshold, true));
   if (c->dbg_wait_hash) HIPCHK(c, hipStreamWaitEvent(c->stream, c->dbg_wait_hash, 0));
+  const bool keyed = keyed_codes(c, W, H, npairs, s);
   CHK(run_hash(c, (const uint8_t*)c->smooth.p, (const uint8_t*)c->grad.p, nullptr, W, H, 2 * npairs, false,
-               (uint32_t*)c->codes.p));
+               (uint32_t*)c->codes.p, 0, 2, nullptr, keyed));
   if (c->dbg_rec_hash) HIPCHK(c, hipEventRecord(c->dbg_rec_hash, c->stream));
-  CHK(run_match(c, W, H, npairs, s, 0, (const uint8_t*)c->grad.p, d_out, cap_per_pair, d_counts, d_ncand));
+  CHK(run_match(c, W, H, npairs, s, 0, (const uint8_t*)c->grad.p, d_out, cap_per_pair, d_counts, d_ncand, nullptr, false, keyed));
   if (c->dbg_rec_join) HIPCHK(c, hipEventRecord(c->dbg_rec_join, c->stream));
   return GPC_OK;
 }
@@ -4438,10 +4486,11 @@
   const size_t n = (size_t)W * H;
   CHK(ensure(c, c->codes, sizeof(uint32_t) * n * 2 * npairs));
   CHK(run_preprocess(c, d_rawL, d_rawR, W, H, npairs, 2, s->gradient_threshold, true));
+  const bool keyed = keyed_codes(c, W, H, npairs, s);
   CHK(run_hash(c, (const uint8_t*)c->smooth.p, (const uint8_t*)c->grad.p, nullptr, W, H, 2 * npairs, false,
-               (uint32_t*)c->codes.p));
+               (uint32_t*)c->codes.p, 0, 2, nullptr, keyed));
   const PackedOut po = {d_rows, (long)cap_per_pair, (long)H};
-  CHK(run_match(c, W, H, npairs, s, 2, (const uint8_t*)c->grad.p, d_packed, cap_per_pair, d_counts, d_ncand, &po));
+  CHK(run_match(c, W, H, npairs, s, 2, (const uint8_t*)c->grad.p, d_packed, cap_per_pair, d_counts, d_ncand, &po, false, keyed));
   return GPC_OK;
 }
 
diff --git a/opengpc_amd/csrc/k_hash.h b/opengpc_amd/csrc/k_hash.h
--- a/opengpc_amd/csrc/k_hash.h
+++ b/opengpc_amd/csrc/k_hash.h
@@ -247,6 +247,20 @@
                                               uint32_t* __restrict__ codes, int W, int H,
                                               const GpcForestDev* __restrict__ fp, int32_t* __restrict__ img_stats,
                                               int tpw, int last_round_from) {
+  constexpr bool KEYED = false;
+#define HT_GROUPS 0
+#include "k_hash_body.h"
+#undef HT_GROUPS
+}
+
+template <bool TAU, int TY = HT_Y>
+__global__ __launch_bounds__(HT_THREADS) HT_OCC void k_hash_keyed(const uint8_t* __restrict__ smooth,
+                                              const uint8_t* __restrict__ grad,
+                                              const uint8_t* __restrict__ candmap,
+                                              uint32_t* __restrict__ codes, int W, int H,
+                                              const GpcForestDev* __restrict__ fp, int32_t* __restrict__ img_stats,
+                                              int tpw, int last_round_from) {
+  constexpr bool DENSE = false, NAIVE = false, GBITS = true, KEYED = true;
 #define HT_GROUPS 0
 #include "k_hash_body.h"
 #undef HT_GROUPS
@@ -267,6 +281,7 @@
                                               uint32_t* __restrict__ codes, int W, int H,
                                               const GpcForestDev* __restrict__ fp_groups, int32_t* __restrict__ img_stats,
                                               int tpw, int last_round_from, int ngroups, int gstep) {
+  constexpr bool KEYED = false;
 #define HT_GROUPS 1
 #include "k_hash_body.h"
 #undef HT_GROUPS
diff --git a/opengpc_amd/csrc/k_hash_body.h b/opengpc_amd/csrc/k_hash_body.h
--- a/opengpc_amd/csrc/k_hash_body.h
+++ b/opengpc_amd/csrc/k_hash_body.h
@@ -106,6 +106,9 @@
   };
 
   constexpr bool INV = !DENSE && !NAIVE;
+  static_assert(!KEYED || INV, "keys are made from the complemented codes of the batched SSE pipelines");
+  constexpr uint32_t KTOP = KEYED ? 0x7F7F7F7Fu : ~0u;
+  constexpr uint32_t KDOM = KEYED ? 0x80000000u : 0u;
   constexpr int CBIT = GBITS ? 0 : 7;
   const int tile0 = by * tpw;
   const int ntiles = (H - 2 * GPC_R + TY - 1) / TY;
@@ -203,7 +206,7 @@
 #pragma unroll
   for (int r = 0; r < RPW; ++r)
 #pragma unroll
-    for (int j = 0; j < 4; ++j) code[r][j] = INV ? ~0u : 0u;
+    for (int j = 0; j < 4; ++j) code[r][j] = INV ? (KEYED ? 0x7FFFFFFFu : ~0u) : 0u;
   HT_STAMP(3);
 
 #ifdef HT_EXP_NOCOMPUTE
@@ -246,8 +249,9 @@
       const uint32_t q0 = INV ? (p0[r] & ((p8[r] >> 7) | ~m8)) : (NAIVE ? ~p0[r] : (~p0[r] | ((~p8[r] >> 7) & m8)));
       const uint32_t q1 = INV ? p1[r] : ~p1[r];
       const uint32_t q2 = INV ? p2[r] : ~p2[r];
-      const uint32_t q3 = INV ? ((p3[r] >> (8 - n3)) | ~m3) : (NAIVE ? ~p3[r] : ((~p3[r] >> (8 - n3)) & m3));
-      if (INV) cor3 = __builtin_amdgcn_bitop3_b32(q3, rowdo[r] ? ~0u : 0u, cor3, 0xAE);
+      const uint32_t q3 = INV ? (KEYED ? __builtin_amdgcn_bitop3_b32(p3[r] >> (8 - n3), m3, KTOP, 0xE2) : ((p3[r] >> (8 - n3)) | ~m3))
+                              : (NAIVE ? ~p3[r] : ((~p3[r] >> (8 - n3)) & m3));
+      if (INV) cor3 = __builtin_amdgcn_bitop3_b32(q3, rowdo[r] ? ~0u : KDOM, cor3, 0xAE);
       const uint32_t lo01 = __builtin_amdgcn_perm(q1, q0, 0x05010400u);
       const uint32_t hi01 = __builtin_amdgcn_perm(q1, q0, 0x07030602u);
       const uint32_t lo23 = __builtin_amdgcn_perm(q3, q2, 0x05010400u);
@@ -275,11 +279,13 @@
           op[j] = (NAIVE && !is_cand) ? 0u : c;
         }
       } else {
-        const uint32_t dom = rowdo[r] ? ~0u : 0u;
+        const uint32_t dom = rowdo[r] ? ~0u : KDOM;
 #pragma unroll
         for (int j = 0; j < 4; ++j) {
           const uint32_t cm4 = (uint32_t)__builtin_amdgcn_sbfe((int)cand8[r], 8 * j + CBIT, 1);
-          if (INV) {
+          if (KEYED) {
+            op[j] = __builtin_amdgcn_bitop3_b32(code[r][j], dom, cm4, 0x08);
+          } else if (INV) {
             op[j] = __builtin_amdgcn_bitop3_b32(code[r][j], dom, cm4, 0x5D);
           } else {
             cor |= code[r][j] & dom;
diff --git a/opengpc_amd/csrc/k_rowjoin_fused.h b/opengpc_amd/csrc/k_rowjoin_fused.h
--- a/opengpc_amd/csrc/k_rowjoin_fused.h
+++ b/opengpc_amd/csrc/k_rowjoin_fused.h
@@ -232,6 +232,11 @@
   return rj_hash(k, shift) | (idx & smask & none);
 }
 
+__device__ __forceinline__ uint32_t rjf_home_keyed(uint32_t k, uint32_t idx, int shift) {
+  const uint32_t rec = (uint32_t)((int32_t)k >> 31);
+  return __builtin_amdgcn_bitop3_b32(rj_hash(k, shift), idx, rec, 0xF4);
+}
+
 constexpr int rjf_log2(int v) {
   int l = 0;
   while ((1 << l) < v) ++l;
@@ -250,8 +255,10 @@
 #ifdef GPC_WGLIFE
 __device__ unsigned long long g_rjf_wg[3 * 4096];
 #endif
-template <int SPT, int NT, bool WIDE>
-__global__ __launch_bounds__(NT) __attribute__((amdgpu_waves_per_eu(8, 8))) void k_row_join_fused(RjfArgs ka) {
+template <int SPT, int NT, bool WIDE, bool KEYED, bool EXACT>
+__device__ __forceinline__ void rjf_rows(const RjfArgs& ka) {
+  static_assert(!KEYED || !WIDE, "keys carry their tag in bit 31: codes below 2^31 only");
+  static_assert(!EXACT || KEYED, "the exact-fit form exists for keyed rows only");
 #ifdef GPC_WGLIFE
   unsigned long long wl_t0;
   unsigned wl_rows = 0u;
@@ -362,9 +369,14 @@
     uint32_t kl[SPT], kr[SPT];
 #pragma unroll
     for (int j = 0; j < SPT; ++j) {
-      const uint32_t inm = (uint32_t)((j * NT + tid - W) >> 31);
-      kl[j] = (ncl[j] + 1u) & inm;
-      kr[j] = (ncr[j] + 1u) & inm;
+      if (KEYED && EXACT) {
+        kl[j] = ncl[j];
+        kr[j] = ncr[j];
+      } else {
+        const uint32_t inm = (uint32_t)((j * NT + tid - W) >> 31);
+        kl[j] = (KEYED ? ncl[j] : ncl[j] + 1u) & inm;
+        kr[j] = (KEYED ? ncr[j] : ncr[j] + 1u) & inm;
+      }
 #ifdef RJ_DBG_EMPTY
       kl[j] = kr[j] = 0u * (ncl[j] + ncr[j]);
 #endif
@@ -408,7 +420,7 @@
       uint32_t old[SPT];
 #pragma unroll
       for (int j = 0; j < SPT; ++j) {
-        h0l[j] = rjf_home(kl[j], (uint32_t)(j * NT + tid), hshift, smask, WIDE);
+        h0l[j] = KEYED ? rjf_home_keyed(kl[j], (uint32_t)(j * NT + tid), hshift) : rjf_home(kl[j], (uint32_t)(j * NT + tid), hshift, smask, WIDE);
         old[j] = atomicMax(&t_key[h0l[j]], kl[j]);
       }
       {
@@ -464,7 +476,7 @@
       uint32_t h0r[SPT], f0l[SPT], f0r[SPT];
 #pragma unroll
       for (int j = 0; j < SPT; ++j) {
-        h0r[j] = rjf_home(kr[j], (uint32_t)(j * NT + tid), hshift, smask, WIDE);
+        h0r[j] = KEYED ? rjf_home_keyed(kr[j], (uint32_t)(j * NT + tid), hshift) : rjf_home(kr[j], (uint32_t)(j * NT + tid), hshift, smask, WIDE);
         f0l[j] = t_key[h0l[j]];
         f0r[j] = t_key[h0r[j]];
       }
@@ -472,8 +484,14 @@
       uint32_t ql[SPT], qr[SPT];
 #pragma unroll
       for (int j = 0; j < SPT; ++j) {
-        ql[j] = WIDE ? kl[j] : (kl[j] | (uint32_t)((int32_t)(kl[j] - 1u) >> 31));
-        qr[j] = WIDE ? kr[j] : (kr[j] | (uint32_t)((int32_t)(kr[j] - 1u) >> 31));
+        if (KEYED) {
+          const uint32_t recl = (uint32_t)((int32_t)kl[j] >> 31), recr = (uint32_t)((int32_t)kr[j] >> 31);
+          ql[j] = __builtin_amdgcn_bitop3_b32(kl[j], recl, recl, 0xF3);
+          qr[j] = __builtin_amdgcn_bitop3_b32(kr[j], recr, recr, 0xF3);
+        } else {
+          ql[j] = WIDE ? kl[j] : (kl[j] | (uint32_t)((int32_t)(kl[j] - 1u) >> 31));
+          qr[j] = WIDE ? kr[j] : (kr[j] | (uint32_t)((int32_t)(kr[j] - 1u) >> 31));
+        }
       }
       {
 #pragma unroll
@@ -510,7 +528,7 @@
         uint32_t kk = WIDE ? (kr[j] ? f0r[j] : 0u) : f0r[j];
         RJF_ASSERT_EXEC_ALL();
         hr[j] = rjf_find_chain(keys_lds, qr[j], kk, h0r[j], smask);
-        const bool hit = WIDE ? (kr[j] && kk == kr[j]) : (kk == qr[j]);
+        const bool hit = WIDE ? (kr[j] && kk == kr[j]) : (kk == (KEYED ? kr[j] : qr[j]));
         mv[j] = (hit ? (F_RSEEN | (uint32_t)(j * NT + tid)) : 0u) << ((hr[j] & 1u) << 4);
       }
 #pragma unroll
@@ -591,7 +609,7 @@
     uint32_t rb[SPT], rs[SPT];
 #pragma unroll
     for (int j = 0; j < SPT; ++j) {
-      rb[j] = (kl[j] - 1u) >> csh;
+      rb[j] = (KEYED ? (kl[j] & 0x7FFFFFFFu) : (kl[j] - 1u)) >> csh;
       rs[j] = 0u;
       if (ok[j]) rs[j] = atomicAdd(&r_cnt[rb[j]], 1u);
     }
@@ -623,7 +641,7 @@
     for (int j = 0; j < SPT; ++j)
       if (ok[j]) {
         rb[j] = r_cnt[rb[j]];
-        if ((rs[j] >> 16) > 1u) r_key[rb[j] + (rs[j] & 0xFFFFu)] = kl[j] - 1u;
+        if ((rs[j] >> 16) > 1u) r_key[rb[j] + (rs[j] & 0xFFFFu)] = KEYED ? kl[j] : kl[j] - 1u;
       }
     __syncthreads();
     RJ_STAMP(5);
@@ -632,7 +650,7 @@
     for (int j = 0; j < SPT; ++j) {
       const bool m = ok[j];
       RJF_ASSERT_EXEC_ALL();
-      const uint32_t rank = rjf_walk(rkey_lds, rb[j], rs[j] >> 16, kl[j] - 1u);
+      const uint32_t rank = rjf_walk(rkey_lds, rb[j], rs[j] >> 16, KEYED ? kl[j] : kl[j] - 1u);
       if (m) d_words[rank] = (uint32_t)(j * NT + tid) | (xr[j] << 16);
     }
     d_pair = pair;
@@ -687,4 +705,14 @@
 #endif
 }
 
-}
+template <int SPT, int NT, bool WIDE>
+__global__ __launch_bounds__(NT) __attribute__((amdgpu_waves_per_eu(8, 8))) void k_row_join_fused(RjfArgs ka) {
+  rjf_rows<SPT, NT, WIDE, false, false>(ka);
+}
+
+template <int SPT, int NT, bool EXACT>
+__global__ __launch_bounds__(NT) __attribute__((amdgpu_waves_per_eu(8, 8))) void k_row_join_fused_keyed(RjfArgs ka) {
+  rjf_rows<SPT, NT, false, true, EXACT>(ka);
+}
+
+}
```

After: 249,800 Mpix/s (median of 6 runs). About the same (+0.5%).
